# AssafSinger94/dino-tracker

Measured on NVIDIA H100. Metric: query-points/sec (854x476, T=50), higher is better.
Workload: dtype f32

## Files before the change

### dino_tracker_b200/csrc/inference.cu

```cuda
#include <algorithm>
#include <vector>

#include "common.cuh"
#include "corr.cuh"
#include "head.cuh"
#include "sample.cuh"
#include "xwin.cuh"

namespace dtk {

constexpr int TC2_BM_ROWS = 256;

__global__ void sample_query_kernel(const float* __restrict__ tpc, int T, int C, int P, int h, int w, PointAffine pa,
                                    const float* __restrict__ qp, float* __restrict__ desc, float* __restrict__ dnorm) {
  int n = blockIdx.x;
  float x = __fadd_rn(__fmul_rn(pa.aw, qp[n * 3 + 0]), pa.bw);
  float y = __fadd_rn(__fmul_rn(pa.ah, qp[n * 3 + 1]), pa.bh);
  int tq = (int)qp[n * 3 + 2];
  tq = min(max(tq, 0), T - 1);
  TriCorners c = tri_setup(x, y, 0.f, 2, h, w);
  sample_point(tpc, C, P, c, tq, -1, desc + (size_t)n * C, dnorm + n);
}

__global__ void index_traj_kernel(const int* __restrict__ grp_frame, const int* __restrict__ grp_row0,
                                  const int* __restrict__ grp_map0, int n_groups, int n_maps, int T,
                                  int* __restrict__ out_index, float* __restrict__ traj) {
  int j = blockIdx.x * blockDim.x + threadIdx.x;
  if (j >= n_maps) return;
  const int lo = last_le(n_groups, j, grp_map0);
  int n = grp_row0[lo] + (j - grp_map0[lo]);
  int t = grp_frame[lo];
  out_index[j] = n * T + t;
  traj[((size_t)n * T + t) * 3 + 2] = (float)t;
}

__global__ void traj_cos_kernel(const float* __restrict__ tpc, int T, int C, int P, int h, int w, PointAffine pa,
                                const float* __restrict__ traj, const float* __restrict__ qp,
                                float* __restrict__ cos_out) {
  extern __shared__ __align__(16) float sm[];
  __shared__ float nrm[2];
  __shared__ float red[SAMPLE_THREADS / 32];
  const int n = blockIdx.y, i = blockIdx.x;
  int tq = (int)qp[n * 3 + 2];
  tq = min(max(tq, 0), T - 1);
  for (int which = 0; which < 2; ++which) {
    const float* pt = traj + ((size_t)n * T + (which == 0 ? tq : i)) * 3;
    float x = __fadd_rn(__fmul_rn(pa.aw, pt[0]), pa.bw);
    float y = __fadd_rn(__fmul_rn(pa.ah, pt[1]), pa.bh);
    TriCorners c = tri_setup(x, y, pt[2], T, h, w);
    sample_point(tpc, C, P, c, c.z0, c.z1, sm + which * C, nrm + which);
    __syncthreads();
  }
  const float nq = fmaxf(nrm[0], 1e-8f), ni = fmaxf(nrm[1], 1e-8f);
  float acc = 0.f;
  for (int c = threadIdx.x; c < C; c += SAMPLE_THREADS) acc = fmaf(__fdiv_rn(sm[c], nq), __fdiv_rn(sm[C + c], ni), acc);
  acc = warp_sum(acc);
  if ((threadIdx.x & 31) == 0) red[threadIdx.x >> 5] = acc;
  __syncthreads();
  if (threadIdx.x == 0) {
    float s = 0.f;
    for (int k = 0; k < SAMPLE_THREADS / 32; ++k) s += red[k];
    cos_out[(size_t)n * T + i] = s;
  }
}

constexpr int ANCHOR_LIST_THREADS = 256;
__global__ void __launch_bounds__(ANCHOR_LIST_THREADS)
anchor_lists_kernel(const float* __restrict__ cos_sims, int N, int T, float th, int* __restrict__ cnt,
                    int* __restrict__ qlist) {
  const int a = blockIdx.x;
  int base = 0;
  for (int n0 = 0; n0 < N; n0 += ANCHOR_LIST_THREADS) {
    const int n = n0 + threadIdx.x;
    const bool v = n < N && cos_sims[(size_t)n * T + a] >= th;
    int total;
    const int rank = block_rank<ANCHOR_LIST_THREADS>(v, &total);
    if (v) qlist[(size_t)a * N + base + rank] = n;
    base += total;
    __syncthreads();
  }
  if (threadIdx.x == 0) cnt[a] = base;
}

struct AnchorItem { int a, slot, i, n; };
__device__ __forceinline__ AnchorItem anchor_item(int j, int lo, int T, const int* __restrict__ qlist, int N,
                                                  const int* __restrict__ grp_frame, const int* __restrict__ grp_map0,
                                                  const int* __restrict__ grp_item0) {
  AnchorItem it;
  it.a = grp_frame[lo];
  const int uu = grp_item0[lo] + (j - grp_map0[lo]);
  it.slot = uu / T; it.i = uu - it.slot * T;
  it.n = qlist[(size_t)it.a * N + it.slot];
  return it;
}

struct NoAnchor {};
__device__ __forceinline__ int slot_frame(int z, int i0, int a) { return z == 0 ? a : i0 + z - 1; }
__device__ __forceinline__ int slot_frame(int z, int i0, NoAnchor) { return i0 + z - 1; }
struct SetSample { TriCorners c; int f0, f1; };
template <class Anchor>
__device__ __forceinline__ SetSample frame_set_sample(const float* __restrict__ pt, int i, int T, int frame_batch, int h, int w,
                                                      const PointAffine& pa, Anchor a) {
  const int i0 = (i / frame_batch) * frame_batch, e = min(i0 + frame_batch, T);
  float x = __fadd_rn(__fmul_rn(pa.aw, pt[0]), pa.bw);
  float y = __fadd_rn(__fmul_rn(pa.ah, pt[1]), pa.bh);
  SetSample s;
  s.c = tri_setup(x, y, (float)(i - i0 + 1), e - i0 + 1, h, w);
  s.f0 = slot_frame(s.c.z0, i0, a);
  s.f1 = s.c.z1 < 0 ? -1 : slot_frame(s.c.z1, i0, a);
  return s;
}

__global__ void sample_anchor_kernel(const float* __restrict__ tpc, int T, int C, int P, int h, int w, PointAffine pa,
                                     const float* __restrict__ traj, const int* __restrict__ qlist, int N,
                                     const int* __restrict__ grp_frame, const int* __restrict__ grp_map0,
                                     const int* __restrict__ grp_item0, int n_groups, int frame_batch,
                                     float* __restrict__ desc, float* __restrict__ dnorm, int* __restrict__ out_index,
                                     __half* __restrict__ desc_hi, __half* __restrict__ desc_lo) {
  const int j = blockIdx.x;
  const AnchorItem it = anchor_item(j, last_le(n_groups, j, grp_map0), T, qlist, N, grp_frame, grp_map0, grp_item0);
  const SetSample s = frame_set_sample(traj + ((size_t)it.n * T + it.i) * 3, it.i, T, frame_batch, h, w, pa, it.a);
  sample_point(tpc, C, P, s.c, s.f0, s.f1, desc + (size_t)j * C, dnorm + j, desc_hi ? desc_hi + (size_t)j * C : nullptr,
               desc_lo ? desc_lo + (size_t)j * C : nullptr);
  if (threadIdx.x == 0) out_index[j] = (it.n * T + it.a) * T + it.i;
}

__device__ __forceinline__ float quant_desc(const __half* hi, const __half* lo, int C, const float* norm, int8_t* q, float* fac) {
  __syncthreads();
  if (threadIdx.x >= 32) return 0.f;
  const float nrm = *norm;
  return xw_quant_row([&](int k) {
    const uint2 a = *reinterpret_cast<const uint2*>(hi + k), b = *reinterpret_cast<const uint2*>(lo + k);
    const float2 a0 = __half22float2(*reinterpret_cast<const __half2*>(&a.x)), a1 = __half22float2(*reinterpret_cast<const __half2*>(&a.y));
    const float2 b0 = __half22float2(*reinterpret_cast<const __half2*>(&b.x)), b1 = __half22float2(*reinterpret_cast<const __half2*>(&b.y));
    return make_float4(a0.x + b0.x, a0.y + b0.y, a1.x + b1.x, a1.y + b1.y);
  }, C, nrm, q, fac);
}

__global__ void sample_unique_kernel(const float* __restrict__ tpc, int T, int C, int P, int h, int w, PointAffine pa,
                                     const float* __restrict__ traj, int frame_batch, __half* __restrict__ u_hi,
                                     __half* __restrict__ u_lo, float* __restrict__ u_norm, int* __restrict__ u_flag,
                                     int8_t* __restrict__ u_q8, float* __restrict__ u_fac, float* __restrict__ u_rho) {
  const int u = blockIdx.x;
  const SetSample s = frame_set_sample(traj + (size_t)u * 3, u % T, T, frame_batch, h, w, pa, NoAnchor{});
  bool slot0 = false;
#pragma unroll
  for (int k = 0; k < 4; ++k) slot0 = slot0 || (s.c.z0 == 0 && s.c.tok[k] >= 0 && s.c.wxy[k][0] != 0.f);
  if (threadIdx.x == 0) u_flag[u] = slot0 ? 1 : 0;
  if (slot0) return;
  sample_point(tpc, C, P, s.c, s.f0, s.f1, nullptr, u_norm + u, u_hi + (size_t)u * C, u_lo + (size_t)u * C);
  if (u_q8) {
    const float r = quant_desc(u_hi + (size_t)u * C, u_lo + (size_t)u * C, C, u_norm + u, u_q8 + (size_t)u * C, u_fac + u);
    if (threadIdx.x == 0) u_rho[u] = r;
  }
}

__global__ void anchor_scalars_kernel(int T, const int* __restrict__ qlist, int N, const int* __restrict__ grp_frame,
                                      const int* __restrict__ grp_row0, const int* __restrict__ grp_map0,
                                      const int* __restrict__ grp_item0, int n_groups, int n_maps, int n_unique, int chunk_row0,
                                      const float* __restrict__ u_norm, const int* __restrict__ u_flag,
                                      const float* __restrict__ u_rho, const float* __restrict__ rho_f, float eps_slack, bool with_eps,
                                      int* __restrict__ out_index, int* __restrict__ arow, float* __restrict__ dnorm,
                                      float* __restrict__ desc_eps) {
  const int j = blockIdx.x * blockDim.x + threadIdx.x;
  if (j >= n_maps) return;
  const int lo = last_le(n_groups, j, grp_map0);
  const AnchorItem it = anchor_item(j, lo, T, qlist, N, grp_frame, grp_map0, grp_item0);
  const size_t u = (size_t)it.n * T + it.i;
  out_index[j] = (it.n * T + it.a) * T + it.i;
  const int r0 = grp_row0[lo];
  arow[j] = r0 < n_unique ? r0 + (j - grp_map0[lo]) : chunk_row0 + j;
  if (u_flag[u]) return;
  dnorm[j] = u_norm[u];
  if (with_eps) desc_eps[j] = xw_eps_s8(u_rho[u], rho_f[it.a], eps_slack);
}

__global__ void gather_anchor_kernel(const float* __restrict__ tpc, int T, int C, int P, int h, int w, PointAffine pa,
                                     const float* __restrict__ traj, const int* __restrict__ qlist, int N,
                                     const int* __restrict__ grp_frame, const int* __restrict__ grp_row0,
                                     const int* __restrict__ grp_map0, const int* __restrict__ grp_item0, int n_groups,
                                     int n_unique, int map_lo, int frame_batch, const __half* __restrict__ u_hi,
                                     const __half* __restrict__ u_lo, const int* __restrict__ u_flag,
                                     float* __restrict__ dnorm, __half* __restrict__ desc_hi,
                                     __half* __restrict__ desc_lo, const int8_t* __restrict__ u_q8,
                                     const float* __restrict__ u_fac, const float* __restrict__ rho_f, float eps_slack,
                                     int8_t* __restrict__ desc_q8, float* __restrict__ desc_fac,
                                     float* __restrict__ desc_eps) {
  const int j = map_lo + blockIdx.x;
  const int lo = last_le(n_groups, j, grp_map0);
  if (grp_row0[lo] < n_unique) return;
  const AnchorItem it = anchor_item(j, lo, T, qlist, N, grp_frame, grp_map0, grp_item0);
  const size_t u = (size_t)it.n * T + it.i;
  if (!u_flag[u]) {
    const uint4* sh = reinterpret_cast<const uint4*>(u_hi + u * C);
    const uint4* sl = reinterpret_cast<const uint4*>(u_lo + u * C);
    uint4* dh = reinterpret_cast<uint4*>(desc_hi + (size_t)j * C);
    uint4* dl = reinterpret_cast<uint4*>(desc_lo + (size_t)j * C);
    for (int k = threadIdx.x; k < C / 8; k += blockDim.x) { dh[k] = __ldg(sh + k); dl[k] = __ldg(sl + k); }
    if (desc_q8) {
      const uint4* sq = reinterpret_cast<const uint4*>(u_q8 + u * C);
      uint4* dq = reinterpret_cast<uint4*>(desc_q8 + (size_t)j * C);
      for (int k = threadIdx.x; k < C / 16; k += blockDim.x) dq[k] = __ldg(sq + k);
      if (threadIdx.x == 0) desc_fac[j] = u_fac[u];
    }
    return;
  }
  const SetSample s = frame_set_sample(traj + u * 3, it.i, T, frame_batch, h, w, pa, it.a);
  sample_point(tpc, C, P, s.c, s.f0, s.f1, nullptr, dnorm + j, desc_hi + (size_t)j * C, desc_lo + (size_t)j * C);
  if (desc_q8) {
    const float r = quant_desc(desc_hi + (size_t)j * C, desc_lo + (size_t)j * C, C, dnorm + j, desc_q8 + (size_t)j * C, desc_fac + j);
    if (threadIdx.x == 0) desc_eps[j] = xw_eps_s8(r, rho_f[it.a], eps_slack);
  }
}

constexpr int OCC_THREADS = 256;
__global__ void occlusion_kernel(const float* __restrict__ traj, const float* __restrict__ cos_sims,
                                 const float* __restrict__ anchors, int T, float anchor_th, float cos_th,
                                 uint8_t* __restrict__ occ) {
  extern __shared__ float sm[];
  float* med = sm;
  int* alist = reinterpret_cast<int*>(sm + T);
  float* ax = sm + 2 * T;
  float* ay = sm + 3 * T;
  const int lane = threadIdx.x & 31, warp = threadIdx.x >> 5, nw = OCC_THREADS / 32;
  float* col = sm + 4 * T + warp * T;
  __shared__ int M;
  __shared__ float th_s;
  const int n = blockIdx.x;
  if (threadIdx.x == 0) {
    int m = 0;
    for (int a = 0; a < T; ++a)
      if (cos_sims[(size_t)n * T + a] >= anchor_th) {
        alist[m] = a;
        ax[m] = traj[((size_t)n * T + a) * 3 + 0];
        ay[m] = traj[((size_t)n * T + a) * 3 + 1];
        ++m;
      }
    M = m;
  }
  __syncthreads();
  const int m = M, want = (m - 1) / 2;
  for (int i = warp; i < T; i += nw) {
    for (int p = lane; p < m; p += 32) {
      const float* g = anchors + (((size_t)n * T + alist[p]) * T + i) * 2;
      float dx = __fsub_rn(g[0], ax[p]), dy = __fsub_rn(g[1], ay[p]);
      col[p] = sqrtf(__fadd_rn(__fmul_rn(dx, dx), __fmul_rn(dy, dy)));
    }
    __syncwarp();
    for (int p = lane; p < m; p += 32) {
      const float dp = col[p];
      int rank = 0;
      for (int q = 0; q < m; ++q) {
        float dq = col[q];
        rank += (dq < dp) || (dq == dp && q < p);
      }
      if (rank == want) med[i] = dp;
    }
    __syncwarp();
  }
  __syncthreads();
  if (threadIdx.x == 0) {
    float th = -INFINITY;
    for (int p = 0; p < m; ++p) th = fmaxf(th, med[alist[p]]);
    th_s = th;
  }
  __syncthreads();
  for (int i = threadIdx.x; i < T; i += blockDim.x)
    occ[(size_t)n * T + i] = (m > 0 && (med[i] > th_s || cos_sims[(size_t)n * T + i] < cos_th)) ? 1 : 0;
}

struct GroupBuf {
  std::vector<int> v;
  int cap, n;
  bool overflow = false;
  explicit GroupBuf(int c) : v((size_t)5 * c), cap(c), n(0) {}
  void clear() { n = 0; }
  void push(int frame, int row0, int m, int map0, int item0) {
    if (n >= cap) { overflow = true; return; }
    v[n] = frame; v[cap + n] = row0; v[2 * cap + n] = m; v[3 * cap + n] = map0; v[4 * cap + n] = item0; ++n;
  }
};

struct ChunkMeta { int used, maxm, n_groups; bool no_thin; int n_gathered, gather_lo, gather_hi; };
constexpr int XW_INPLACE_PAD_DIV = 16;
constexpr int XW_INPLACE_MIN_ROWS = TC2_BM_ROWS - TC2_BM_ROWS / (XW_INPLACE_PAD_DIV + 1);
struct AnchorRows { const int* qlist; const unsigned char* qflag; int gather_row0, ring, ring_stride; };
static bool plan_chunks(int kind, int T, int N, const int* cnt, int ch_all, int gcap, std::vector<ChunkMeta>& metas,
                        std::vector<int>& plan_host, int align = 1, int first_cap = 0, const AnchorRows* rows = nullptr) {
  int ch = ch_all;
  metas.clear(); plan_host.clear();
  GroupBuf gb(gcap);
  int n_gathered = 0, gather_lo = 0, gather_hi = 0;
  auto commit_chunk = [&](int used) {
    bool no_thin = true;
    int maxm = 0;
    for (int k = 0; k < gb.n; ++k) {
      no_thin = no_thin && gb.v[2 * gb.cap + k] > STREAM_MAX_M;
      maxm = std::max(maxm, gb.v[2 * gb.cap + k]);
    }
    metas.push_back(ChunkMeta{used, maxm, gb.n, no_thin, n_gathered, gather_lo, gather_hi});
    plan_host.insert(plan_host.end(), gb.v.begin(), gb.v.end());
    n_gathered = gather_lo = gather_hi = 0;
  };
  auto push_span = [&](int a, int map0, int m, int item0) {
    if (!rows) { gb.push(a, map0, m, map0, item0); return; }
    const int* ql = rows->qlist + (size_t)a * N;
    const int chunk_row0 = rows->gather_row0 + (int)(metas.size() % rows->ring) * rows->ring_stride;
    const int s0 = item0 / T, s1 = (item0 + m) / T;
    int gs = -1;
    auto close_gathered = [&](int s_end) {
      if (gs < 0) return;
      const int gm = (s_end - gs) * T, gmap = map0 + (gs - s0) * T;
      gb.push(a, chunk_row0 + gmap, gm, gmap, gs * T);
      if (n_gathered == 0) gather_lo = gmap;
      n_gathered += gm; gather_hi = gmap + gm;
      gs = -1;
    };
    for (int s = s0; s < s1;) {
      const bool flagged = rows->qflag[ql[s]] != 0;
      int e = s + 1;
      while (!flagged && e < s1 && ql[e] == ql[e - 1] + 1 && !rows->qflag[ql[e]]) ++e;
      const int r = (e - s) * T, pad = (r + TC2_BM_ROWS - 1) / TC2_BM_ROWS * TC2_BM_ROWS - r;
      if (!flagged && (long long)pad * XW_INPLACE_PAD_DIV <= r) {
        close_gathered(s);
        gb.push(a, ql[s] * T, r, map0 + (s - s0) * T, s * T);
      } else if (gs < 0) {
        gs = s;
      }
      s = e;
    }
    close_gathered(s1);
  };
  if (kind == 0) {
    int t = 0, row = 0;
    while (t < T) {
      gb.clear();
      int used = 0;
      while (t < T && used < ch && gb.n < gcap) {
        int m = N - row;
        if (m > ch - used) m = ch - used;
        gb.push(t, row, m, used, 0);
        used += m; row += m;
        if (row == N) { row = 0; ++t; }
      }
      commit_chunk(used);
    }
  } else {
    int a = 0;
    long long item = 0;
    while (a < T) {
      gb.clear();
      int used = 0;
      ch = (metas.empty() && first_cap > 0 && first_cap < ch_all) ? first_cap : ch_all;
      while (a < T && used < ch && gb.n < gcap) {
        long long tot = (long long)cnt[a] * T;
        long long m = tot - item;
        if (m > ch - used) {
          m = (long long)((ch - used) / align) * align;
          if (m == 0 && used > 0) break;
          if (m == 0) m = align;
        }
        if (m > 0) {
          push_span(a, used, (int)m, (int)item);
          used += (int)m; item += m;
        }
        if (item >= tot) { item = 0; ++a; }
      }
      if (used == 0) break;
      commit_chunk(used);
    }
  }
  return !gb.overflow;
}

struct CellPlan {
  std::vector<int> v;
  std::vector<size_t> first;
  std::vector<int> tiles;
  int max_m = 0;
};
static void plan_cells(int T, int gcap, const std::vector<ChunkMeta>& metas, const std::vector<int>& plan_host, CellPlan& cp) {
  const int nb = (T + XW_MAX_CELL - 1) / XW_MAX_CELL, rb = (T + nb - 1) / nb;
  cp.v.clear(); cp.first.assign(1, 0); cp.tiles.clear(); cp.max_m = 0;
  std::vector<int> r0, mm, fr, gr, ar;
  for (size_t k = 0; k < metas.size(); ++k) {
    const int* gb = plan_host.data() + k * 5 * gcap;
    r0.clear(); mm.clear(); fr.clear(); gr.clear(); ar.clear();
    int pre = 0;
    for (int g = 0; g < metas[k].n_groups; ++g) {
      const int frame = gb[g], row0 = gb[gcap + g], m = gb[2 * gcap + g], map0 = gb[3 * gcap + g];
      cp.tiles.push_back(pre);
      pre += (m + TC2_BM_ROWS - 1) / TC2_BM_ROWS;
      for (int s0 = 0; s0 < m; s0 += T)
        for (int b = 0; b < T; b += rb) {
          const int cm = std::min(rb, T - b);
          r0.push_back(map0 + s0 + b); mm.push_back(cm); fr.push_back(frame); gr.push_back(g); ar.push_back(row0 + s0 + b);
          cp.max_m = std::max(cp.max_m, cm);
        }
    }
    for (int g = metas[k].n_groups; g <= gcap; ++g) cp.tiles.push_back(pre);
    const size_t n = r0.size();
    cp.v.insert(cp.v.end(), r0.begin(), r0.end());
    cp.v.insert(cp.v.end(), mm.begin(), mm.end());
    cp.v.insert(cp.v.end(), fr.begin(), fr.end());
    cp.v.insert(cp.v.end(), gr.begin(), gr.end());
    cp.v.insert(cp.v.end(), ar.begin(), ar.end());
    cp.first.push_back(cp.first.back() + n);
  }
}

struct InferAsync {
  cudaStream_t side;
  cudaEvent_t fork, join, sample[2], gemm[2];
};
static int g_overlap_mode = -1;
struct InferAsyncSlot { InferAsync ia; int state; };
static InferAsync* infer_async() {
  static PerDev<InferAsyncSlot> slots;
  if (g_overlap_mode == 0) return nullptr;
  InferAsyncSlot& slot = slots.get();
  InferAsync& ia = slot.ia;
  if (slot.state == 0) {
    slot.state = -1;
    if (cudaStreamCreateWithFlags(&ia.side, cudaStreamNonBlocking) != cudaSuccess) return nullptr;
    cudaEvent_t* evs[] = {&ia.fork, &ia.join, &ia.sample[0], &ia.sample[1], &ia.gemm[0], &ia.gemm[1]};
    for (cudaEvent_t* ev : evs)
      if (cudaEventCreateWithFlags(ev, cudaEventDisableTiming) != cudaSuccess) return nullptr;
    slot.state = 1;
  }
  return slot.state == 1 ? &ia : nullptr;
}

constexpr int XW_RING = 4;
constexpr int XW_PROBE_MAPS = 4096;
constexpr int INFER_A_COUNTED = 16;
constexpr int XW_CNT_CHUNK = 4, XW_CNT_A = XW_CNT_CHUNK * XW_RING, XW_CNT_MINNORM = XW_CNT_A + INFER_A_COUNTED;
struct XwAsync {
  int state;
  cudaEvent_t sample[XW_RING], done[XW_RING], freed[XW_RING];
  int* host_cnt;
};
static XwAsync* xw_async() {
  static PerDev<XwAsync> slots;
  XwAsync& xa = slots.get();
  if (xa.state == 0) {
    xa.state = -1;
    for (int k = 0; k < XW_RING; ++k) {
      if (cudaEventCreateWithFlags(&xa.sample[k], cudaEventDisableTiming) != cudaSuccess) return nullptr;
      if (cudaEventCreateWithFlags(&xa.done[k], cudaEventDisableTiming) != cudaSuccess) return nullptr;
      if (cudaEventCreateWithFlags(&xa.freed[k], cudaEventDisableTiming) != cudaSuccess) return nullptr;
    }
    if (cudaHostAlloc(&xa.host_cnt, (XW_CNT_MINNORM + 4) * sizeof(int), cudaHostAllocDefault) != cudaSuccess) return nullptr;
    xa.state = 1;
  }
  return xa.state == 1 ? &xa : nullptr;
}
static int g_xw_path = -1;
static int g_xw_coarse = -1;
namespace infer_stat {
enum { anchor_maps, exact_window, full_map, pipeline, full_map_by_certificate, contraction, coarse, coarse_rho_f,
       desc_in_place, desc_gathered, exact_box_cells, exact_box_tokens, count };
}
static long long g_infer_stats[infer_stat::count] = {};
constexpr int XW_S8_PROBE_QUEUE_DIV = 16;

struct AnchorChoice {
  XwAsync* xa = nullptr;
  bool xw = false;
  bool probe = false;
  bool s8 = false;

  AnchorChoice(const FeatView& fv, const dinotrk_geom& g) {
    if (fv.tensor() && disc_fits_box(g) && g_xw_path != 0) xa = xw_async();
    xw = xa != nullptr;
    probe = g_xw_path < 0;
  }
  static bool q8_rows(const FeatView& fv) { return fv.s8() && g_xw_coarse != 0 && fv.C % 16 == 0 && fv.C <= XW_S8_MAX_C; }
  void after_sync(int C, int n_counted_A, long long maps_A) {
    if (!xw) return;
    float mn;
    memcpy(&mn, xa->host_cnt + XW_CNT_MINNORM, sizeof(float));
    if (!(mn >= split_min_norm(C))) xw = false;
    if (xw && probe && n_counted_A > 0) {
      long long unc = 0;
      for (int k = 0; k < n_counted_A; ++k) unc += xa->host_cnt[XW_CNT_A + k];
      if (unc * 4 > maps_A) xw = false;
    }
  }
  int coarse_pass(const FeatView& fv, float rho_max) {
    DTK_CHECK_ARG(g_xw_coarse != 1 || !xw || fv.s8(), "infer: int8 coarse pass forced without the int8 features");
    s8 = xw && fv.s8() && g_xw_coarse != 0;
    DTK_CHECK_ARG(!s8 || (fv.C % 16 == 0 && fv.C <= XW_S8_MAX_C), "infer: int8 coarse pass needs C %% 16 == 0 and C <= %d",
                  XW_S8_MAX_C);
    if (g_xw_coarse < 0 && !(rho_max <= XW_S8_RHO_MAX)) s8 = false;
    return DINOTRK_OK;
  }
  bool probe_says_full_maps(long long by_certificate, long long queued, int maps) {
    if (by_certificate * 4 > maps) return true;
    if (s8 && g_xw_coarse < 0 && queued * XW_S8_PROBE_QUEUE_DIV > maps) s8 = false;
    return false;
  }
};

struct CorrTrackWs {
  float* maps; CorrMapsWs corr; int* hscratch;
  CorrTrackWs(Arena& ar, int total_maps, int n_groups, int C, int map_stride)
      : maps(ar.take<float>((size_t)total_maps * map_stride)), corr(ar, total_maps, n_groups, C),
        hscratch(ar.take<int>(total_maps + 1)) {}
};

struct ChunkBufs {
  float* maps; float* desc; float* norm; int* plan; float* split; int* hscratch; unsigned long long* tkeys;
  ChunkBufs() = default;
  ChunkBufs(Arena& ar, int C, int N, int P, int ms, int ch, int gcap) {
    maps = ar.take<float>((size_t)ch * ms);
    desc = ar.take<float>((size_t)ch * C);
    norm = ar.take<float>(ch);
    plan = ar.take<int>(gcap + 1);
    split = ar.take<float>(corr_tc_workspace_bytes(ch > N ? ch : N, C) / 4);
    hscratch = ar.take<int>(ch + 1);
    tkeys = ar.take<unsigned long long>((size_t)ch * cdiv(P, CORR_TILE));
  }
};

struct XwSet {
  int row0; float* norm; int* out_index; int* arow; float* eps; XwChunk xc;
  XwSet() = default;
  XwSet(Arena& ar, int row0_, float* u_norm, int P, int ch, int gcap) : row0(row0_), norm(u_norm + row0_) {
    out_index = ar.take<int>(ch);
    arow = ar.take<int>(ch);
    eps = ar.take<float>(ch);
    xc = XwChunk(ar, ch, (size_t)ch + 2, cdiv(P, XW_TILE), gcap);
  }
};

struct InferWs {
  float* descA; float* normA;
  ChunkBufs cb[2];
  int* out_index_ring[4];
  int* d_groups; int* d_cnt; int* d_qlist;
  size_t xw_rows;
  __half* u_hi; __half* u_lo; int8_t* u_q8; float* u_norm; float* u_fac; int* u_flag; float* u_rho;
  float* d_rnorms; unsigned* d_minnorm;
  XwSet xr[XW_RING];
  int cell_nb;
  int* d_cells; int* d_tiles;
  int sg_cap;
  int* d_cgrp; int* d_splan; int* d_cntA;
  InferWs(Arena& ar, int T, int C, int N, int P, int ms, int ch, int gcap, size_t max_chunks) {
    descA = ar.take<float>((size_t)N * C);
    normA = ar.take<float>(N);
    for (ChunkBufs& b : cb) b = ChunkBufs(ar, C, N, P, ms, ch, gcap);
    for (int*& r : out_index_ring) r = ar.take<int>(ch);
    d_groups = ar.take<int>(max_chunks * 5 * gcap);
    d_cnt = ar.take<int>(T);
    d_qlist = ar.take<int>((size_t)T * N);
    const int n_unique = N * T;
    xw_rows = (size_t)n_unique + (size_t)XW_RING * ch;
    u_hi = ar.take<__half>(xw_rows * C);
    u_lo = ar.take<__half>(xw_rows * C);
    u_q8 = ar.take<int8_t>(xw_rows * C);
    u_norm = ar.take<float>(xw_rows);
    u_fac = ar.take<float>(xw_rows);
    u_flag = ar.take<int>((size_t)N * T);
    u_rho = ar.take<float>((size_t)N * T);
    d_rnorms = ar.take<float>((size_t)T * P);
    d_minnorm = ar.take<unsigned>(4);
    for (int k = 0; k < XW_RING; ++k) xr[k] = XwSet(ar, n_unique + k * ch, u_norm, P, ch, gcap);
    cell_nb = (T + XW_MAX_CELL - 1) / XW_MAX_CELL;
    d_cells = ar.take<int>((size_t)N * T * cell_nb * 5 + 16);
    d_tiles = ar.take<int>(max_chunks * (gcap + 1));
    sg_cap = (int)std::min<size_t>(max_chunks * (size_t)gcap, 16384);
    d_cgrp = ar.take<int>((size_t)4 * sg_cap);
    d_splan = ar.take<int>((size_t)sg_cap + 1);
    d_cntA = ar.take<int>(64);
  }
};

struct InferCtx {
  const FeatView& fv; const dinotrk_geom& g; const dinotrk_head_weights& hw;
  InferWs& ws; cudaStream_t st;
  int T, C, N, P, ms, ch, gcap, fb;
  size_t max_chunks;
  PointAffine pa;
  std::vector<ChunkMeta> metas;
  std::vector<int> plan_host;
  int upload_plan() {
    DTK_CHECK_ARG(metas.size() <= max_chunks, "infer: chunk plan exceeds its bound (%zu > %zu)", metas.size(), max_chunks);
    if (!plan_host.empty())
      DTK_CUDA(cudaMemcpyAsync(ws.d_groups, plan_host.data(), plan_host.size() * sizeof(int), cudaMemcpyHostToDevice, st));
    return DINOTRK_OK;
  }
  struct Grp { const int *f, *r, *m, *map0, *item; };
  Grp grp_of(size_t k) const {
    const int* b = ws.d_groups + k * 5 * gcap;
    return Grp{b, b + gcap, b + 2 * gcap, b + 3 * gcap, b + 4 * gcap};
  }
};

static int infer_trajectories(InferCtx& c, const float* query_points, float* traj, int& n_counted) {
  NvtxRange nv("dinotrk.infer.A.trajectories");
  InferWs& ws = c.ws;
  const bool tensor = c.fv.tensor();
  {
    ProfRange pr(PROF_SAMPLE, c.st);
    sample_query_kernel<<<c.N, SAMPLE_THREADS, 0, c.st>>>(c.fv.tpc, c.T, c.C, c.P, c.g.h, c.g.w, c.pa, query_points, ws.descA,
                                                           ws.normA);
    DTK_LAUNCHED();
  }
  if (tensor) {
    for (int k = 0; k < 2; ++k) {
      const DescSplit a(ws.cb[k].split, c.N, c.C);
      int rc = corr_hilo(c.fv) ? launch_split_hilo(ws.descA, a.hi, c.N, c.C, c.st)
                               : launch_split_f16(ws.descA, a.hi, a.lo, (size_t)c.N * c.C, c.st);
      if (rc) return rc;
    }
  }
  plan_chunks(0, c.T, c.N, nullptr, c.ch, c.gcap, c.metas, c.plan_host);
  int rc = c.upload_plan();
  if (rc) return rc;
  for (size_t k = 0; k < c.metas.size(); ++k) {
    const ChunkMeta& cm = c.metas[k];
    const ChunkBufs& b = ws.cb[k & 1];
    const InferCtx::Grp gp = c.grp_of(k);
    {
      ProfRange pr(PROF_MISC, c.st);
      index_traj_kernel<<<cdiv(cm.used, 256), 256, 0, c.st>>>(gp.f, gp.r, gp.map0, cm.n_groups, cm.used, c.T,
                                                              ws.out_index_ring[k & 3], traj);
      DTK_LAUNCHED();
    }
    CorrAssist as;
    as.tkeys = tensor ? b.tkeys : nullptr; as.zero_word = b.hscratch; as.split_ready = tensor; as.no_thin = cm.no_thin;
    rc = launch_corr_maps(c.fv, ws.descA, c.N, ws.normA, gp.f, gp.r, gp.m, gp.map0, cm.n_groups, cm.used, cm.maxm, b.maps, c.ms,
                          b.plan, b.split, c.st, as);
    if (rc) return rc;
    rc = launch_head(b.maps, cm.used, c.ms, c.g, c.hw, ws.out_index_ring[k & 3], traj, 3, 0, nullptr, b.hscratch, c.st, as.tkeys,
                     true);
    if (rc) return rc;
    if (k < INFER_A_COUNTED)
      DTK_CUDA(cudaMemcpyAsync(ws.d_cntA + k, b.hscratch, sizeof(int), cudaMemcpyDeviceToDevice, c.st));
  }
  n_counted = (int)std::min<size_t>(c.metas.size(), INFER_A_COUNTED);
  return DINOTRK_OK;
}

struct ExactWindow {
  InferCtx& c;
  const AnchorChoice& choice;
  const CellPlan& cp;
  bool ovl;
  cudaStream_t sb;
  const float* traj;
  float* anchors;
  int q_rows = 0, q_groups = 0;

  XwCells cells_of(size_t k) const {
    XwCells x;
    const int n = (int)(cp.first[k + 1] - cp.first[k]);
    const int* base = c.ws.d_cells + 5 * cp.first[k];
    x.row0 = base; x.m = base + n; x.frame = base + 2 * n; x.group = base + 3 * n; x.arow = base + 4 * n;
    x.n_cells = n; x.max_m = cp.max_m;
    return x;
  }
  int sample(size_t k) {
    InferWs& ws = c.ws;
    const ChunkMeta& cm = c.metas[k];
    const XwSet& x = ws.xr[k % XW_RING];
    const InferCtx::Grp gp = c.grp_of(k);
    if (ovl && k >= XW_RING) DTK_CUDA(cudaStreamWaitEvent(sb, choice.xa->freed[k % XW_RING], 0));
    {
      ProfRange pr(PROF_SAMPLE, sb);
      anchor_scalars_kernel<<<cdiv(cm.used, 256), 256, 0, sb>>>(c.T, ws.d_qlist, c.N, gp.f, gp.r, gp.map0, gp.item, cm.n_groups,
                                                               cm.used, c.N * c.T, x.row0, ws.u_norm, ws.u_flag, ws.u_rho,
                                                               c.fv.q_rho, xw_s8_slack(c.C), choice.s8, x.out_index, x.arow,
                                                               x.norm, x.eps);
      DTK_LAUNCHED();
      if (cm.n_gathered > 0) {
        const size_t r0 = (size_t)x.row0;
        gather_anchor_kernel<<<cm.gather_hi - cm.gather_lo, SAMPLE_THREADS, 0, sb>>>(
            c.fv.tpc, c.T, c.C, c.P, c.g.h, c.g.w, c.pa, traj, ws.d_qlist, c.N, gp.f, gp.r, gp.map0, gp.item, cm.n_groups,
            c.N * c.T, cm.gather_lo, c.fb, ws.u_hi, ws.u_lo, ws.u_flag, x.norm, ws.u_hi + r0 * c.C, ws.u_lo + r0 * c.C, ws.u_q8,
            ws.u_fac, c.fv.q_rho, xw_s8_slack(c.C), choice.s8 ? ws.u_q8 + r0 * c.C : nullptr, ws.u_fac + r0, x.eps);
        DTK_LAUNCHED();
      }
    }
    if (ovl) DTK_CUDA(cudaEventRecord(choice.xa->sample[k % XW_RING], sb));
    return DINOTRK_OK;
  }
  int flush() {
    if (q_rows == 0) return DINOTRK_OK;
    const ChunkBufs& b = c.ws.cb[0];
    CorrAssist as;
    as.tkeys = b.tkeys; as.zero_word = b.hscratch; as.split_ready = true; as.no_thin = true; as.all_wide = true; as.small_tiles = true;
    const int* cg = c.ws.d_cgrp;
    const int sg = c.ws.sg_cap;
    int rc = launch_corr_maps(c.fv, nullptr, c.ch, b.norm, cg, cg + sg, cg + 2 * sg, cg + 3 * sg, q_groups, q_rows, q_rows,
                              b.maps, c.ms, c.ws.d_splan, b.split, c.st, as);
    if (rc) return rc;
    rc = launch_head(b.maps, q_rows, c.ms, c.g, c.hw, c.ws.out_index_ring[0], anchors, 2, 0, nullptr, b.hscratch, c.st, b.tkeys,
                     true);
    q_rows = q_groups = 0;
    return rc;
  }
  int finish(size_t j) {
    InferWs& ws = c.ws;
    XwAsync* xa = choice.xa;
    DTK_CUDA(cudaEventSynchronize(xa->done[j % XW_RING]));
    const int* cnt = xa->host_cnt + XW_CNT_CHUNK * (j % XW_RING);
    const int n_slow = cnt[0];
    g_infer_stats[infer_stat::full_map_by_certificate] += cnt[1];
    g_infer_stats[infer_stat::exact_box_tokens] += cnt[2]; g_infer_stats[infer_stat::exact_box_cells] += cnt[3];
    const ChunkMeta& cm = c.metas[j];
    const XwSet& x = ws.xr[j % XW_RING];
    const InferCtx::Grp gp = c.grp_of(j);
    DTK_CHECK_ARG(n_slow >= 0 && n_slow <= cm.used, "infer: corrupt full-map queue (%d of %d)", n_slow, cm.used);
    g_infer_stats[infer_stat::exact_window] += cm.used - n_slow; g_infer_stats[infer_stat::full_map] += n_slow;
    if (n_slow > 0) {
      if (q_rows + n_slow > c.ch || q_groups + cm.n_groups > ws.sg_cap) {
        int rc = flush();
        if (rc) return rc;
      }
      const ChunkBufs& b = ws.cb[0];
      const DescSplit d(b.split, c.ch, c.C);
      int rc = launch_xw_compact(nullptr, ws.u_hi, ws.u_lo, x.arow, x.norm, x.out_index, c.C, gp.f, gp.map0, cm.n_groups, n_slow,
                                 x.xc, nullptr, d.hi, d.lo, b.norm, ws.out_index_ring[0], ws.d_cgrp, ws.sg_cap, c.st, q_rows,
                                 q_groups, corr_hilo(c.fv));
      if (rc) return rc;
      q_rows += n_slow; q_groups += cm.n_groups;
    }
    DTK_CUDA(cudaEventRecord(xa->freed[j % XW_RING], c.st));
    return DINOTRK_OK;
  }
};

static int anchors_exact_window(InferCtx& c, AnchorChoice& choice, const float* traj, float* anchors, size_t& done) {
  InferWs& ws = c.ws;
  const cudaStream_t st = c.st;
  XwAsync* xa = choice.xa;
  CellPlan cp;
  plan_cells(c.T, c.gcap, c.metas, c.plan_host, cp);
  DTK_CHECK_ARG(cp.first.back() * 5 <= (size_t)c.N * c.T * ws.cell_nb * 5 + 16, "infer: cell plan exceeds its bound");
  if (!cp.v.empty()) DTK_CUDA(cudaMemcpyAsync(ws.d_cells, cp.v.data(), cp.v.size() * sizeof(int), cudaMemcpyHostToDevice, st));
  if (!cp.tiles.empty()) DTK_CUDA(cudaMemcpyAsync(ws.d_tiles, cp.tiles.data(), cp.tiles.size() * sizeof(int), cudaMemcpyHostToDevice, st));
  InferAsync* ia = infer_async();
  const bool ovl = ia != nullptr && c.metas.size() > 1;
  ExactWindow pipe{c, choice, cp, ovl, ovl ? ia->side : st, traj, anchors};
  if (ovl) {
    DTK_CUDA(cudaEventRecord(ia->fork, st));
    DTK_CUDA(cudaStreamWaitEvent(pipe.sb, ia->fork, 0));
  }
  int rc;
  if (!c.metas.empty() && (rc = pipe.sample(0))) return rc;
  size_t n_finished = 0;
  done = c.metas.size();
  for (size_t k = 0; k < c.metas.size(); ++k) {
    const ChunkMeta& cm = c.metas[k];
    const XwSet& x = ws.xr[k % XW_RING];
    const InferCtx::Grp gp = c.grp_of(k);
    const XwCells cells = pipe.cells_of(k);
    if (ovl) DTK_CUDA(cudaStreamWaitEvent(st, xa->sample[k % XW_RING], 0));
    const float* eps = choice.s8 ? x.eps : nullptr;
    g_infer_stats[infer_stat::desc_in_place] += cm.used - cm.n_gathered; g_infer_stats[infer_stat::desc_gathered] += cm.n_gathered;
    if ((rc = launch_xw_coarse(c.fv, ws.u_hi, (int)ws.xw_rows, ws.u_norm, gp.f, gp.r, gp.m, gp.map0, ws.d_tiles + k * (c.gcap + 1),
                               cm.n_groups, cm.used / TC2_BM_ROWS + cm.n_groups, x.xc, st, ws.d_rnorms,
                               choice.s8 ? ws.u_q8 : nullptr, ws.u_fac))) return rc;
    if ((rc = launch_xw_plan(cells, x.norm, cm.n_groups, c.g, x.xc, st, cm.used, split_min_norm(c.C), eps))) return rc;
    if ((rc = launch_xw_gemm(c.fv, c.g, ws.u_hi, ws.u_lo, (int)ws.xw_rows, cells, x.xc, st))) return rc;
    if ((rc = launch_xw_head(c.fv, c.g, c.hw, cells, x.norm, gp.map0, cm.used, x.out_index, anchors, 2, 0, x.xc, st, cm.n_groups,
                             eps)))
      return rc;
    DTK_CUDA(cudaMemcpyAsync(xa->host_cnt + XW_CNT_CHUNK * (k % XW_RING), x.xc.slow_cnt + cm.n_groups, XW_CNT_CHUNK * sizeof(int),
                             cudaMemcpyDeviceToHost, st));
    DTK_CUDA(cudaEventRecord(xa->done[k % XW_RING], st));
    if (k == 0 && choice.probe && c.metas.size() > 1) {
      if ((rc = pipe.finish(0))) return rc;
      n_finished = 1;
      if (choice.probe_says_full_maps(g_infer_stats[infer_stat::full_map_by_certificate], g_infer_stats[infer_stat::full_map], cm.used)) {
        done = 1;
        break;
      }
      g_infer_stats[infer_stat::coarse] = choice.s8 ? 1 : 0;
    }
    if (k + 1 < c.metas.size() && (rc = pipe.sample(k + 1))) return rc;
    while (n_finished + 2 <= k)
      if ((rc = pipe.finish(n_finished++))) return rc;
  }
  while (n_finished < done)
    if ((rc = pipe.finish(n_finished++))) return rc;
  if ((rc = pipe.flush())) return rc;
  if (ovl) {
    DTK_CUDA(cudaEventRecord(ia->join, pipe.sb));
    DTK_CUDA(cudaStreamWaitEvent(st, ia->join, 0));
  }
  return DINOTRK_OK;
}

static int anchors_full_map(InferCtx& c, size_t k0, const float* traj, float* anchors) {
  InferWs& ws = c.ws;
  const cudaStream_t st = c.st;
  const bool tensor = c.fv.tensor();
  FeatView fv_split = c.fv;
  fv_split.hilo = nullptr;
  InferAsync* ia = infer_async();
  const bool ovl = ia != nullptr && c.metas.size() > k0 + 1;
  const cudaStream_t sb = ovl ? ia->side : st;
  if (ovl) {
    DTK_CUDA(cudaEventRecord(ia->fork, st));
    DTK_CUDA(cudaStreamWaitEvent(sb, ia->fork, 0));
  }
  auto sample = [&](size_t k) -> int {
    const ChunkMeta& cm = c.metas[k];
    const ChunkBufs& b = ws.cb[k & 1];
    const InferCtx::Grp gp = c.grp_of(k);
    if (ovl && k >= k0 + 2) DTK_CUDA(cudaStreamWaitEvent(sb, ia->gemm[k & 1], 0));
    {
      ProfRange pr(PROF_SAMPLE, sb);
      const DescSplit d(b.split, cm.used, c.C);
      __half* d_hi = tensor ? reinterpret_cast<__half*>(d.hi) : nullptr;
      __half* d_lo = tensor ? reinterpret_cast<__half*>(d.lo) : nullptr;
      sample_anchor_kernel<<<cm.used, SAMPLE_THREADS, 0, sb>>>(c.fv.tpc, c.T, c.C, c.P, c.g.h, c.g.w, c.pa, traj, ws.d_qlist, c.N,
                                                              gp.f, gp.map0, gp.item, cm.n_groups, c.fb, b.desc, b.norm,
                                                              ws.out_index_ring[k & 3], d_hi, d_lo);
      DTK_LAUNCHED();
    }
    if (ovl) DTK_CUDA(cudaEventRecord(ia->sample[k & 1], sb));
    return DINOTRK_OK;
  };
  auto head_full = [&](size_t j) {
    const ChunkBufs& b = ws.cb[j & 1];
    return launch_head(b.maps, c.metas[j].used, c.ms, c.g, c.hw, ws.out_index_ring[j & 3], anchors, 2, 0, nullptr, b.hscratch,
                       st, tensor ? b.tkeys : nullptr, true, 2);
  };
  int rc;
  if (k0 < c.metas.size() && (rc = sample(k0))) return rc;
  for (size_t k = k0; k < c.metas.size(); ++k) {
    const ChunkMeta& cm = c.metas[k];
    const ChunkBufs& b = ws.cb[k & 1];
    const InferCtx::Grp gp = c.grp_of(k);
    if (ovl) DTK_CUDA(cudaStreamWaitEvent(st, ia->sample[k & 1], 0));
    if (k >= k0 + 2 && (rc = head_full(k - 2))) return rc;
    CorrAssist as;
    as.tkeys = tensor ? b.tkeys : nullptr; as.zero_word = b.hscratch; as.split_ready = tensor; as.no_thin = cm.no_thin;
    rc = launch_corr_maps(fv_split, b.desc, cm.used, b.norm, gp.f, gp.r, gp.m, gp.map0, cm.n_groups, cm.used, cm.maxm, b.maps,
                          c.ms, b.plan, b.split, st, as);
    if (rc) return rc;
    if (ovl) DTK_CUDA(cudaEventRecord(ia->gemm[k & 1], st));
    if (k + 1 < c.metas.size() && (rc = sample(k + 1))) return rc;
    rc = launch_head(b.maps, cm.used, c.ms, c.g, c.hw, ws.out_index_ring[k & 3], anchors, 2, 0, nullptr, b.hscratch, st, as.tkeys,
                     true, 1);
    if (rc) return rc;
  }
  for (size_t j = std::max(k0, c.metas.size() >= 2 ? c.metas.size() - 2 : 0); j < c.metas.size(); ++j)
    if ((rc = head_full(j))) return rc;
  return DINOTRK_OK;
}

static int infer_anchors(InferCtx& c, const float* traj, const float* cos_sims, float anchor_th, float* anchors, int n_counted_A) {
  NvtxRange nv("dinotrk.infer.C.anchors");
  InferWs& ws = c.ws;
  const cudaStream_t st = c.st;
  const int T = c.T, N = c.N;
  {
    ProfRange pr(PROF_ANCHOR_LIST, st);
    anchor_lists_kernel<<<T, ANCHOR_LIST_THREADS, 0, st>>>(cos_sims, N, T, anchor_th, ws.d_cnt, ws.d_qlist);
    DTK_LAUNCHED();
  }
  AnchorChoice choice(c.fv, c.g);
  XwAsync* xa = choice.xa;
  if (xa) {
    int rc = launch_xw_rnorms(c.fv, ws.d_rnorms, ws.d_minnorm, st);
    if (rc) return rc;
    DTK_CUDA(cudaMemcpyAsync(xa->host_cnt + XW_CNT_MINNORM, ws.d_minnorm, sizeof(unsigned), cudaMemcpyDeviceToHost, st));
    if (n_counted_A > 0)
      DTK_CUDA(cudaMemcpyAsync(xa->host_cnt + XW_CNT_A, ws.d_cntA, (size_t)n_counted_A * sizeof(int), cudaMemcpyDeviceToHost, st));
  }
  std::vector<int> cnt(T);
  DTK_CUDA(cudaMemcpyAsync(cnt.data(), ws.d_cnt, (size_t)T * sizeof(int), cudaMemcpyDeviceToHost, st));
  std::vector<float> rho_f(c.fv.s8() ? T : 0);
  if (c.fv.s8()) DTK_CUDA(cudaMemcpyAsync(rho_f.data(), c.fv.q_rho, (size_t)T * sizeof(float), cudaMemcpyDeviceToHost, st));
  std::vector<int> qlist_h, uflag_h;
  if (choice.xw) {
    {
      ProfRange pr(PROF_SAMPLE, st);
      sample_unique_kernel<<<N * T, SAMPLE_THREADS, 0, st>>>(c.fv.tpc, T, c.C, c.P, c.g.h, c.g.w, c.pa, traj, c.fb, ws.u_hi, ws.u_lo,
                                                             ws.u_norm, ws.u_flag, AnchorChoice::q8_rows(c.fv) ? ws.u_q8 : nullptr,
                                                             ws.u_fac, ws.u_rho);
      DTK_LAUNCHED();
    }
    qlist_h.resize((size_t)T * N); uflag_h.resize((size_t)N * T);
    DTK_CUDA(cudaMemcpyAsync(qlist_h.data(), ws.d_qlist, qlist_h.size() * sizeof(int), cudaMemcpyDeviceToHost, st));
    DTK_CUDA(cudaMemcpyAsync(uflag_h.data(), ws.u_flag, uflag_h.size() * sizeof(int), cudaMemcpyDeviceToHost, st));
  }
  DTK_CUDA(cudaStreamSynchronize(st));
  choice.after_sync(c.C, n_counted_A, (long long)N * T);
  long long maps_C = 0;
  for (int a = 0; a < T; ++a) maps_C += (long long)cnt[a] * T;
  long long* stats = g_infer_stats;
  stats[infer_stat::anchor_maps] = maps_C; stats[infer_stat::exact_window] = 0; stats[infer_stat::full_map] = 0;
  stats[infer_stat::pipeline] = choice.xw ? 1 : 0; stats[infer_stat::full_map_by_certificate] = 0;
  stats[infer_stat::contraction] = c.fv.tensor() ? 1 : 0; stats[infer_stat::desc_in_place] = 0; stats[infer_stat::desc_gathered] = 0;
  stats[infer_stat::exact_box_cells] = 0; stats[infer_stat::exact_box_tokens] = 0;
  float rho_max = 0.f;
  for (float r : rho_f) rho_max = std::max(rho_max, r);
  int rc = choice.coarse_pass(c.fv, rho_max);
  if (rc) return rc;
  unsigned bits;
  memcpy(&bits, &rho_max, sizeof(bits));
  stats[infer_stat::coarse] = choice.s8 ? 1 : 0; stats[infer_stat::coarse_rho_f] = bits;
  const int probe_cap = choice.probe ? std::max(T, (XW_PROBE_MAPS / T) * T) : 0;
  size_t k0 = 0;
  if (choice.xw) {
    std::vector<unsigned char> qflag(N, 0);
    for (size_t u = 0; u < uflag_h.size(); ++u)
      if (uflag_h[u]) qflag[u / T] = 1;
    const AnchorRows rows{qlist_h.data(), qflag.data(), N * T, XW_RING, c.ch};
    DTK_CHECK_ARG(plan_chunks(1, T, N, cnt.data(), c.ch, c.gcap, c.metas, c.plan_host, T, probe_cap, &rows),
                  "infer: a chunk of the anchor phase has more than %d groups", c.gcap);
    if ((rc = c.upload_plan())) return rc;
    if ((rc = anchors_exact_window(c, choice, traj, anchors, k0))) return rc;
    if (k0 == c.metas.size()) return DINOTRK_OK;
    stats[infer_stat::pipeline] = 0; stats[infer_stat::coarse] = 0;
    plan_chunks(1, T, N, cnt.data(), c.ch, c.gcap, c.metas, c.plan_host, T, probe_cap);
  } else {
    plan_chunks(1, T, N, cnt.data(), c.ch, c.gcap, c.metas, c.plan_host);
  }
  if ((rc = c.upload_plan())) return rc;
  return anchors_full_map(c, k0, traj, anchors);
}

}

using namespace dtk;

extern "C" {

int dinotrk_infer_set_path(int path) {
  DTK_CHECK_ARG(path >= -1 && path <= 1, "infer_set_path: -1 (automatic), 0 (full-map GEMM + head) or 1 (coarse pass + exact window)");
  g_xw_path = path;
  return DINOTRK_OK;
}

int dinotrk_infer_set_coarse(int mode) {
  DTK_CHECK_ARG(mode >= -1 && mode <= 1, "infer_set_coarse: -1 (automatic), 0 (fp16) or 1 (int8)");
  g_xw_coarse = mode;
  return DINOTRK_OK;
}

int dinotrk_infer_last_stats(long long* out, int n) {
  DTK_CHECK_ARG(out && n >= 4, "infer_last_stats: need at least 4 slots");
  for (int i = 0; i < (n < infer_stat::count ? n : infer_stat::count); ++i) out[i] = g_infer_stats[i];
  return DINOTRK_OK;
}

static int infer_chunk_maps(int chunk_maps) { return chunk_maps > 0 ? chunk_maps : 4096; }
static int infer_chunk_eff(int chunk_maps, int T) { const int c = infer_chunk_maps(chunk_maps); return c > T ? c : T; }
static int infer_gcap(int T, int ch) { return T + 2 + 2 * (ch / XW_INPLACE_MIN_ROWS + 1); }
static size_t infer_max_chunks(int T, int N, size_t ch) {
  size_t cap = (ch / (size_t)T) * (size_t)T;
  if (cap < (size_t)T) cap = T;
  return ((size_t)N * T * T + cap - 1) / cap + 2;
}

size_t dinotrk_infer_max_chunks(int T, int N, int chunk_maps) {
  const size_t ch = (size_t)infer_chunk_maps(chunk_maps);
  return ((size_t)N * T * T + ch - 1) / ch + 2;
}

int dinotrk_infer_plan(int kind, int T, int N, const int* anchor_counts, int chunk_maps, int* groups, int* meta,
                       int max_chunks, int* n_chunks) {
  DTK_CHECK_ARG((kind == 0 || kind == 1) && T > 0 && N >= 0 && n_chunks, "infer_plan: bad arguments");
  DTK_CHECK_ARG(kind == 0 || anchor_counts, "infer_plan: kind 1 needs the per-frame anchor counts");
  const int ch = infer_chunk_maps(chunk_maps), gcap = T + 2;
  std::vector<ChunkMeta> metas;
  std::vector<int> plan_host;
  plan_chunks(kind, T, N, anchor_counts, ch, gcap, metas, plan_host);
  *n_chunks = (int)metas.size();
  DTK_CHECK_ARG((int)metas.size() <= max_chunks || (!groups && !meta), "infer_plan: %zu chunks, room for %d", metas.size(), max_chunks);
  if (groups) std::copy(plan_host.begin(), plan_host.end(), groups);
  if (meta)
    for (size_t k = 0; k < metas.size(); ++k) {
      meta[4 * k] = metas[k].used; meta[4 * k + 1] = metas[k].maxm; meta[4 * k + 2] = metas[k].n_groups;
      meta[4 * k + 3] = metas[k].no_thin ? 1 : 0;
    }
  return DINOTRK_OK;
}

int dinotrk_infer_anchor_gcap(int T, int chunk_maps) { return T > 0 ? infer_gcap(T, infer_chunk_eff(chunk_maps, T)) : 0; }

int dinotrk_infer_plan_anchors(int T, int N, const int* anchor_counts, const int* qlist, const unsigned char* query_flag,
                               int chunk_maps, int probe, int* groups, int* meta, int max_chunks, int* n_chunks) {
  DTK_CHECK_ARG(T > 0 && N >= 0 && anchor_counts && qlist && query_flag && n_chunks, "infer_plan_anchors: bad arguments");
  for (int a = 0; a < T; ++a) {
    DTK_CHECK_ARG(anchor_counts[a] >= 0 && anchor_counts[a] <= N, "infer_plan_anchors: count of frame %d out of range", a);
    for (int k = 0; k < anchor_counts[a]; ++k)
      DTK_CHECK_ARG(qlist[(size_t)a * N + k] >= 0 && qlist[(size_t)a * N + k] < N, "infer_plan_anchors: query out of range");
  }
  const int ch = infer_chunk_eff(chunk_maps, T), gcap = infer_gcap(T, ch);
  const AnchorRows rows{qlist, query_flag, N * T, XW_RING, ch};
  std::vector<ChunkMeta> metas;
  std::vector<int> plan_host;
  const bool fits = plan_chunks(1, T, N, anchor_counts, ch, gcap, metas, plan_host, T,
                                probe ? std::max(T, (XW_PROBE_MAPS / T) * T) : 0, &rows);
  DTK_CHECK_ARG(fits, "infer_plan_anchors: a chunk has more than %d groups", gcap);
  *n_chunks = (int)metas.size();
  DTK_CHECK_ARG((int)metas.size() <= max_chunks || (!groups && !meta), "infer_plan_anchors: %zu chunks, room for %d", metas.size(), max_chunks);
  if (groups) std::copy(plan_host.begin(), plan_host.end(), groups);
  if (meta)
    for (size_t k = 0; k < metas.size(); ++k) {
      meta[5 * k] = metas[k].used; meta[5 * k + 1] = metas[k].maxm; meta[5 * k + 2] = metas[k].n_groups;
      meta[5 * k + 3] = metas[k].no_thin ? 1 : 0; meta[5 * k + 4] = metas[k].n_gathered;
    }
  return DINOTRK_OK;
}

int dinotrk_infer_set_overlap(int mode) {
  DTK_CHECK_ARG(mode >= -1 && mode <= 1, "infer_set_overlap: mode must be -1 (default), 0 or 1");
  g_overlap_mode = mode;
  return DINOTRK_OK;
}

size_t dinotrk_corr_track_workspace_bytes(int total_maps, int n_groups, int C, const dinotrk_geom* g) {
  if (!g) return 0;
  return align_up(layout_end<CorrTrackWs>(total_maps, n_groups, C, dinotrk_map_stride(g)), 256) + 1024;
}

int dinotrk_corr_track(const dinotrk_features* feat, const dinotrk_geom* g,
                       const dinotrk_head_weights* hw, const float* desc, const float* desc_norm,
                       const int* grp_frame, const int* grp_row0, const int* grp_m, const int* grp_map0,
                       int n_groups, int total_maps, int max_group_m, const int* out_index, float* out,
                       int out_stride, int out_mode, void* workspace, size_t workspace_bytes, void* stream) {
  DTK_CHECK_ARG(feat && feat->tpc && feat->norms && g && hw && desc && desc_norm && grp_frame && grp_row0 && grp_m &&
                grp_map0 && out, "corr_track: null pointer");
  const int C = feat->C;
  DTK_CHECK_ARG(feat->T > 0 && C > 0 && C % 4 == 0 && n_groups >= 0 && total_maps >= 0, "corr_track: bad sizes");
  DTK_CHECK_ARG((feat->hi == nullptr) == (feat->lo == nullptr), "corr_track: hi and lo must be given together");
  DTK_CHECK_ARG(workspace && workspace_bytes >= dinotrk_corr_track_workspace_bytes(total_maps, n_groups, C, g),
                "corr_track: workspace too small");
  if (total_maps == 0) return DINOTRK_OK;
  const int ms = dinotrk_map_stride(g);
  Arena ar(workspace);
  const CorrTrackWs ws(ar, total_maps, n_groups, C, ms);
  cudaStream_t st = (cudaStream_t)stream;
  int rc = launch_corr_maps(make_view(*feat, *g), desc, total_maps, desc_norm, grp_frame, grp_row0, grp_m, grp_map0,
                            n_groups, total_maps, max_group_m, ws.maps, ms, ws.corr.plan, ws.corr.split, st);
  if (rc) return rc;
  return launch_head(ws.maps, total_maps, ms, *g, *hw, out_index, out, out_stride, out_mode, nullptr, ws.hscratch, st);
}


size_t dinotrk_infer_workspace_bytes(int T, int C, const dinotrk_geom* g, int N, int chunk_maps) {
  if (!g) return 0;
  const int ch = infer_chunk_eff(chunk_maps, T);
  const size_t end = layout_end<InferWs>(T, C, N, g->h * g->w, dinotrk_map_stride(g), ch, infer_gcap(T, ch),
                                         infer_max_chunks(T, N, (size_t)ch));
  return align_up(end, 256) + 25088;
}

int dinotrk_traj_cos_sims(const float* tpc, int T, int C, const dinotrk_geom* g, const float* traj,
                          const float* query_points, int N, float* cos_sims, void* workspace,
                          size_t workspace_bytes, void* stream) {
  (void)workspace; (void)workspace_bytes;
  DTK_CHECK_ARG(tpc && g && traj && query_points && cos_sims, "traj_cos_sims: null pointer");
  DTK_CHECK_ARG(T > 0 && C > 0 && C % 4 == 0 && N >= 0, "traj_cos_sims: bad sizes");
  if (N == 0) return DINOTRK_OK;
  size_t smem = (size_t)2 * C * sizeof(float);
  static PerDev<size_t> attr_dev;
  size_t& attr = attr_dev.get();
  if (smem > 48 * 1024 && smem > attr) {
    DTK_CUDA(cudaFuncSetAttribute(traj_cos_kernel, cudaFuncAttributeMaxDynamicSharedMemorySize, (int)smem));
    attr = smem;
  }
  ProfRange pr(PROF_COS, (cudaStream_t)stream);
  traj_cos_kernel<<<dim3(T, N), SAMPLE_THREADS, smem, (cudaStream_t)stream>>>(
      tpc, T, C, g->h * g->w, g->h, g->w, make_point_affine(*g), traj, query_points, cos_sims);
  DTK_LAUNCHED();
  return DINOTRK_OK;
}

int dinotrk_occlusion(const float* traj, const float* cos_sims, const float* anchors, int N, int T,
                      float anchor_th, float cos_th, uint8_t* occ, void* stream) {
  DTK_CHECK_ARG(traj && cos_sims && anchors && occ && N >= 0 && T > 0, "occlusion: bad args");
  if (N == 0) return DINOTRK_OK;
  size_t smem = (size_t)(4 + OCC_THREADS / 32) * T * sizeof(float);
  DTK_CHECK_ARG(smem <= 200 * 1024, "occlusion: T=%d too large", T);
  static PerDev<size_t> attr_dev;
  size_t& attr = attr_dev.get();
  if (smem > 48 * 1024 && smem > attr) {
    DTK_CUDA(cudaFuncSetAttribute(occlusion_kernel, cudaFuncAttributeMaxDynamicSharedMemorySize, (int)smem));
    attr = smem;
  }
  ProfRange pr(PROF_OCCLUSION, (cudaStream_t)stream);
  occlusion_kernel<<<N, OCC_THREADS, smem, (cudaStream_t)stream>>>(traj, cos_sims, anchors, T, anchor_th, cos_th, occ);
  DTK_LAUNCHED();
  return DINOTRK_OK;
}

int dinotrk_infer(const dinotrk_features* feat, const dinotrk_geom* g,
                  const dinotrk_head_weights* hw, const float* query_points, int N, float anchor_th, float cos_th,
                  int frame_batch, int start_phase, int stop_after, int chunk_maps, float* traj, float* cos_sims,
                  float* anchors,
                  uint8_t* occ, void* workspace, size_t workspace_bytes, void* stream) {
  DTK_CHECK_ARG(feat && feat->tpc && feat->norms && g && hw && query_points && traj, "infer: null pointer");
  const int T = feat->T, C = feat->C;
  DTK_CHECK_ARG(T > 0 && C > 0 && C % 4 == 0 && N >= 0, "infer: bad sizes");
  DTK_CHECK_GRID(*g, "infer");
  DTK_CHECK_ARG((feat->hi == nullptr) == (feat->lo == nullptr), "infer: hi and lo must be given together");
  const FeatView fv = make_view(*feat, *g);
  DTK_CHECK_ARG(start_phase >= 0 && start_phase <= stop_after && stop_after <= 3,
                "infer: need 0 <= start_phase <= stop_after <= 3");
  DTK_CHECK_ARG((stop_after < 1 || cos_sims) && (stop_after < 2 || anchors) && (stop_after < 3 || occ),
                "infer: missing output buffer for the requested phases");
  DTK_CHECK_ARG(workspace && workspace_bytes >= dinotrk_infer_workspace_bytes(T, C, g, N, chunk_maps),
                "infer: workspace too small (%zu < %zu)", workspace_bytes,
                dinotrk_infer_workspace_bytes(T, C, g, N, chunk_maps));
  if (N == 0) return DINOTRK_OK;
  const int P = g->h * g->w, ms = dinotrk_map_stride(g);
  const int ch = infer_chunk_eff(chunk_maps, T);
  const int fb = frame_batch > 0 ? (frame_batch < T ? frame_batch : T) : T;
  const int gcap = infer_gcap(T, ch);
  const size_t max_chunks = infer_max_chunks(T, N, (size_t)ch);
  Arena ar(workspace);
  InferWs ws(ar, T, C, N, P, ms, ch, gcap, max_chunks);
  DTK_CHECK_ARG(ws.xw_rows <= 0x7fffffffu, "infer: %zu descriptor rows exceed the row index", ws.xw_rows);
  InferCtx c{fv, *g, *hw, ws, (cudaStream_t)stream, T, C, N, P, ms, ch, gcap, fb, max_chunks, make_point_affine(*g)};

  int rc, n_counted_A = 0;
  if (start_phase <= 0 && (rc = infer_trajectories(c, query_points, traj, n_counted_A))) return rc;
  if (stop_after < 1) return DINOTRK_OK;
  if (start_phase <= 1) {
    NvtxRange nv("dinotrk.infer.B.cos_sims");
    if ((rc = dinotrk_traj_cos_sims(feat->tpc, T, C, g, traj, query_points, N, cos_sims, nullptr, 0, stream))) return rc;
  }
  if (stop_after < 2) return DINOTRK_OK;
  if (start_phase <= 2 && (rc = infer_anchors(c, traj, cos_sims, anchor_th, anchors, n_counted_A))) return rc;
  if (stop_after < 3) return DINOTRK_OK;
  NvtxRange nv("dinotrk.infer.D.occlusion");
  return dinotrk_occlusion(traj, cos_sims, anchors, N, T, anchor_th, cos_th, occ, stream);
}

}
```

### dino_tracker_b200/csrc/xwin.cu

```cuda
#include <cuda_fp16.h>

#include "common.cuh"
#include "corr.cuh"
#include "head.cuh"
#include "tcgemm.cuh"
#include "xwin.cuh"

namespace dtk {

constexpr int XW_GEMM_BN = 2 * XW_TILE;

template <class Acc>
struct CoarseEpi {
  static constexpr bool kFragment = true;
  static constexpr bool kS8 = std::is_same<Acc, int>::value;
  const float* rnorms;
  const float* desc_norm;
  const int* grp_map0;
  unsigned long long* key1;
  float* max2;
  int n_tiles, P;

  struct Pre { float2 col; float dv; int map0; };
  __device__ __forceinline__ Pre begin(const TcTile& tl, int t, int r) const {
    const float* rn = rnorms + (size_t)tl.batch * P;
    const int c0 = tl.n0 + t, c1 = c0 + XW_TILE;
    const int rr = r + 8 * ((threadIdx.x & 3) >> 1);
    Pre p;
    p.col = make_float2(c0 < P ? __ldg(rn + c0) : 0.f, c1 < P ? __ldg(rn + c1) : 0.f);
    p.dv = rr < tl.m ? __ldg(desc_norm + tl.row0 + rr) : 0.f;
    p.map0 = __ldg(grp_map0 + tl.g);
    return p;
  }
  static __device__ __forceinline__ float as_float(Acc a) {
    if constexpr (kS8) return __int_as_float(a); else return a;
  }
  static __device__ __forceinline__ Acc from_float(float v) {
    if constexpr (kS8) return __float_as_int(v); else return v;
  }
  template <bool EDGE>
  __device__ __forceinline__ void fold_max(float (&m1)[2], int kh, const float* cols, int n0, int fc,
                                           Acc (&acc)[XW_GEMM_BN / 2]) const {
#pragma unroll
    for (int ii = 0; ii < XW_TILE / 8; ++ii) {
      const int i = kh * XW_TILE / 8 + ii;
      const float2 rnv = tc::lds_f2(tc::smem_u32(cols + fc + 8 * i));
      const int col = n0 + 8 * i + fc;
      const bool ok0 = !EDGE || col < P, ok1 = !EDGE || col + 1 < P;
#pragma unroll
      for (int h = 0; h < 2; ++h) {
        const float a = ok0 ? (float)acc[4 * i + 2 * h] * rnv.x : -INFINITY;
        const float b = ok1 ? (float)acc[4 * i + 2 * h + 1] * rnv.y : -INFINITY;
        acc[4 * i + 2 * h] = from_float(a);
        acc[4 * i + 2 * h + 1] = from_float(b);
        m1[h] = fmaxf(m1[h], fmaxf(a, b));
      }
    }
  }
  __device__ __forceinline__ void scan(float m1, int h, int kh, const Acc (&acc)[XW_GEMM_BN / 2], float& pos,
                                       float& m2) const {
    pos = 0.f;
    m2 = -INFINITY;
#pragma unroll
    for (int ii = XW_TILE / 8 - 1; ii >= 0; --ii) {
      const int i = kh * XW_TILE / 8 + ii;
#pragma unroll
      for (int j = 1; j >= 0; --j)
        asm("{\n\t.reg .pred p;\n\t"
            "setp.eq.f32 p, %2, %3;\n\t"
            "@p fma.rn.f32 %0, %0, 0f3B000000, %4;\n\t"
            "@!p max.f32 %1, %1, %2;\n\t}"
            : "+f"(pos), "+f"(m2)
            : "f"(as_float(acc[4 * i + 2 * h + j])), "f"(m1), "f"((float)(8 * i + j + 1)));
    }
  }
  __device__ __forceinline__ void fragment(const TcTile& tl, int r, int fc, Acc (&acc)[XW_GEMM_BN / 2], const float* cols,
                                           const Pre& pre) const {
    const int q = threadIdx.x & 3, n0 = tl.n0;
    const bool edge = n0 + XW_GEMM_BN > P;
    float o1, o2;
    int otok;
#pragma unroll
    for (int kh = 0; kh < 2; ++kh) {
      float m1[2] = {-INFINITY, -INFINITY};
      if (edge) fold_max<true>(m1, kh, cols, n0, fc, acc);
      else fold_max<false>(m1, kh, cols, n0, fc, acc);
#pragma unroll
      for (int h = 0; h < 2; ++h) {
#pragma unroll
        for (int sh = 1; sh <= 2; sh <<= 1) m1[h] = fmaxf(m1[h], __shfl_xor_sync(0xffffffffu, m1[h], sh));
        float pos, m2;
        scan(m1[h], h, kh, acc, pos, m2);
        const int ip = (int)pos;
        int tok = ip ? n0 + fc + ip - 1 : 0x7fffffff;
        int cnt = (ip != 0) + ((float)ip != pos);
#pragma unroll
        for (int sh = 1; sh <= 2; sh <<= 1) {
          tok = min(tok, __shfl_xor_sync(0xffffffffu, tok, sh));
          cnt += __shfl_xor_sync(0xffffffffu, cnt, sh);
          m2 = fmaxf(m2, __shfl_xor_sync(0xffffffffu, m2, sh));
        }
        if ((q & 1) == kh && (q >> 1) == h) {
          o1 = m1[h];
          o2 = cnt > 1 ? m1[h] : m2;
          otok = tok;
        }
      }
    }
    const int rr = r + 8 * (q >> 1), nt = n0 / XW_TILE + (q & 1);
    if (rr >= tl.m || nt >= n_tiles) return;
    const float rdn = kS8 ? pre.dv : __fdividef(1.f, fmaxf(pre.dv, XW_MIN_NORM));
    const size_t off = (size_t)(pre.map0 + rr) * n_tiles + nt;
    key1[off] = ((unsigned long long)__float_as_uint(fmaxf(o1 * rdn, 0.f)) << 32) | (unsigned)(0x7fffffff - otok);
    max2[off] = fmaxf(o2 * rdn, 0.f);
  }
};

__global__ void xw_rnorm_kernel(const float* __restrict__ norms, float* __restrict__ rnorms, size_t n, unsigned* __restrict__ min_bits) {
  float mn = INFINITY;
  for (size_t i = (size_t)blockIdx.x * blockDim.x + threadIdx.x; i < n; i += (size_t)gridDim.x * blockDim.x) {
    const float v = norms[i];
    rnorms[i] = __fdiv_rn(1.f, fmaxf(v, XW_MIN_NORM));
    mn = fminf(mn, v);
  }
#pragma unroll
  for (int o = 16; o > 0; o >>= 1) mn = fminf(mn, __shfl_xor_sync(0xffffffffu, mn, o));
  if ((threadIdx.x & 31) == 0) atomicMin(min_bits, __float_as_uint(fmaxf(mn, 0.f)));
}

int launch_xw_rnorms(const FeatView& fv, float* rnorms, unsigned* min_bits, cudaStream_t st) {
  const size_t n = (size_t)fv.T * fv.P;
  DTK_CUDA(cudaMemsetAsync(min_bits, 0x7f, sizeof(unsigned), st));
  ProfRange pr(PROF_XW_PLAN, st);
  xw_rnorm_kernel<<<num_sms() * 4, 256, 0, st>>>(fv.norms, rnorms, n, min_bits);
  DTK_LAUNCHED();
  return DINOTRK_OK;
}

int launch_xw_coarse(const FeatView& fv, const void* desc_hi, int desc_rows, const float* desc_norm, const int* grp_frame,
                     const int* grp_row0, const int* grp_m, const int* grp_map0, const int* tile_start, int n_groups,
                     int max_tiles, const XwChunk& xc, cudaStream_t st, const float* rnorms, const void* desc_q8,
                     const float* desc_fac) {
  static_assert(XW_GEMM_BN == 256 && XW_TILE == 128, "one m64n256 GEMM N tile = two 128-token key tiles (CoarseEpi::fragment)");
  TcProblem pb{grp_frame, grp_row0, grp_m, tile_start, n_groups, fv.P, fv.C};
  if (desc_q8) {
    DTK_CHECK_ARG(fv.s8() && fv.C % 16 == 0 && fv.C <= XW_S8_MAX_C, "int8 coarse pass: needs the int8 features, C %% 16 == 0 "
                  "and C <= %d", XW_S8_MAX_C);
    CoarseEpi<int> epi{fv.q_fac, desc_fac, grp_map0, xc.key1, xc.max2, cdiv(fv.P, XW_TILE), fv.P};
    return tc_launch<TcMode::S8, CoarseEpi<int>, XW_GEMM_BN, true>({desc_q8, nullptr, (uint64_t)desc_rows, 0, fv.q8, nullptr,
                                                                    (uint64_t)fv.T, 0}, pb, max_tiles, epi, st, PROF_XW_COARSE);
  }
  CoarseEpi<float> epi{rnorms, desc_norm, grp_map0, xc.key1, xc.max2, cdiv(fv.P, XW_TILE), fv.P};
  return tc_launch<TcMode::F16, CoarseEpi<float>, XW_GEMM_BN, true>({desc_hi, nullptr, (uint64_t)desc_rows, 0, fv.hi, nullptr,
                                                                     (uint64_t)fv.T, 0}, pb, max_tiles, epi, st, PROF_XW_COARSE);
}

constexpr int PLAN_WARPS = 8;
template <int KPL>
__global__ void __launch_bounds__(PLAN_WARPS * 32)
xw_cand_kernel(int n_maps, const float* __restrict__ desc_norm, float min_norm, int n_groups, int n_tiles,
               const unsigned long long* __restrict__ key1, const float* __restrict__ eps_map,
               const float* __restrict__ max2, int* __restrict__ cand, int* __restrict__ pinfo, int* __restrict__ slow_cnt) {
  const int lane = threadIdx.x & 31;
  const int gw = blockIdx.x * PLAN_WARPS + (threadIdx.x >> 5), nw = gridDim.x * PLAN_WARPS;
  if (gw == 0)
    for (int i = lane; i <= n_groups + 3; i += 32) slow_cnt[i] = 0;
  for (int map = gw; map < n_maps; map += nw) {
    const unsigned long long* k1 = key1 + (size_t)map * n_tiles;
    const float* k2 = max2 + (size_t)map * n_tiles;
    unsigned long long kk[KPL] = {};
    float v2[KPL] = {};
#pragma unroll
    for (int q = 0; q < KPL; ++q) {
      const int t = lane + 32 * q;
      if (t < n_tiles) { kk[q] = __ldg(k1 + t); v2[q] = __ldg(k2 + t); }
    }
    unsigned long long gk = kk[0];
#pragma unroll
    for (int q = 1; q < KPL; ++q) gk = gk > kk[q] ? gk : kk[q];
#pragma unroll
    for (int o = 16; o > 0; o >>= 1) { unsigned long long t = __shfl_xor_sync(0xffffffffu, gk, o); gk = t > gk ? t : gk; }
    const float gmax = __uint_as_float((unsigned)(gk >> 32));
    const int ptok = 0x7fffffff - (int)(gk & 0xffffffffu);
    const float eps = eps_map ? eps_map[map] : XW_EPS;
    const float th = gmax - 2.f * eps;
    bool amb = false;
    int ncand = 0;
#pragma unroll
    for (int q = 0; q < KPL; ++q) {
      const int t = lane + 32 * q;
      const bool in = t < n_tiles;
      const bool isc = in && __uint_as_float((unsigned)(kk[q] >> 32)) >= th;
      const unsigned cm = __ballot_sync(0xffffffffu, isc);
      amb = amb || __any_sync(0xffffffffu, in && v2[q] >= th);
      const int rank = ncand + __popc(cm & ((1u << lane) - 1u));
      if (isc && rank < XW_MAX_CAND) cand[(size_t)map * XW_MAX_CAND + rank] = 0x7fffffff - (int)(kk[q] & 0xffffffffu);
      ncand += __popc(cm);
    }
    amb = amb || ncand > XW_MAX_CAND || !(gmax > 4.f * eps) || !(desc_norm[map] >= min_norm);
    if (lane >= ncand && lane < XW_MAX_CAND) cand[(size_t)map * XW_MAX_CAND + lane] = -1;
    if (lane == 0) pinfo[map] = amb ? -1 - ptok : ptok;
  }
}

__global__ void __launch_bounds__(PLAN_WARPS * 32)
xw_cell_kernel(XwCells cells, int w, const int* __restrict__ cand, const int* __restrict__ pinfo, int* __restrict__ stat,
               int* __restrict__ cell_of, int2* __restrict__ box_org, int4* __restrict__ box_ext, int* __restrict__ box_cnt) {
  __shared__ short s_r[PLAN_WARPS][XW_MAX_CELL], s_c[PLAN_WARPS][XW_MAX_CELL];
  __shared__ unsigned char s_ok[PLAN_WARPS][XW_MAX_CELL];
  const int lane = threadIdx.x & 31, wid = threadIdx.x >> 5;
  const int gw = blockIdx.x * PLAN_WARPS + wid, nw = gridDim.x * PLAN_WARPS;
  for (int cell = gw; cell < cells.n_cells; cell += nw) {
    const int row0 = cells.row0[cell], m = cells.m[cell];
    int nv = 0;
    for (int r = lane; r < m; r += 32) {
      const int pi = __ldg(pinfo + row0 + r);
      const int ptok = pi >= 0 ? pi : -1 - pi;
      s_r[wid][r] = (short)(ptok / w);
      s_c[wid][r] = (short)(ptok - (ptok / w) * w);
      s_ok[wid][r] = pi >= 0 ? 1 : 0;
      nv += pi >= 0 ? 1 : 0;
      cell_of[row0 + r] = cell;
    }
    __syncwarp();
#pragma unroll
    for (int o = 16; o > 0; o >>= 1) nv += __shfl_xor_sync(0xffffffffu, nv, o);
    int med_r = -1, med_c = -1;
    if (nv > 0) {
      const int want = (nv - 1) / 2;
      for (int r = lane; r < m; r += 32) {
        if (!s_ok[wid][r]) continue;
        int rk_r = 0, rk_c = 0;
        const int vr = s_r[wid][r], vc = s_c[wid][r];
        for (int q = 0; q < m; ++q) {
          if (!s_ok[wid][q]) continue;
          rk_r += (s_r[wid][q] < vr) || (s_r[wid][q] == vr && q < r);
          rk_c += (s_c[wid][q] < vc) || (s_c[wid][q] == vc && q < r);
        }
        if (rk_r == want) med_r = vr;
        if (rk_c == want) med_c = vc;
      }
#pragma unroll
      for (int o = 16; o > 0; o >>= 1) {
        med_r = max(med_r, __shfl_xor_sync(0xffffffffu, med_r, o));
        med_c = max(med_c, __shfl_xor_sync(0xffffffffu, med_c, o));
      }
    }
    int n_fit = 0, lo_r = INT_MAX, hi_r = INT_MIN, lo_c = INT_MAX, hi_c = INT_MIN;
    for (int r = lane; r < m; r += 32) {
      const int map = row0 + r;
      bool fit = s_ok[wid][r] != 0;
      int mr0 = INT_MAX, mr1 = INT_MIN, mc0 = INT_MAX, mc1 = INT_MIN;
      if (fit) {
        const int4 cd = __ldg(reinterpret_cast<const int4*>(cand) + map);
        const int ct[4] = {cd.x, cd.y, cd.z, cd.w};
#pragma unroll
        for (int q = 0; q < XW_MAX_CAND; ++q)
          if (ct[q] >= 0) {
            const int tr = ct[q] / w, tc_ = ct[q] - tr * w;
            fit = fit && abs(tr - med_r) <= XW_SLACK && abs(tc_ - med_c) <= XW_SLACK;
            mr0 = min(mr0, tr); mr1 = max(mr1, tr); mc0 = min(mc0, tc_); mc1 = max(mc1, tc_);
          }
      }
      stat[map] = fit ? 0 : 1;
      n_fit += fit ? 1 : 0;
      if (fit) { lo_r = min(lo_r, mr0); hi_r = max(hi_r, mr1); lo_c = min(lo_c, mc0); hi_c = max(hi_c, mc1); }
    }
#pragma unroll
    for (int o = 16; o > 0; o >>= 1) {
      n_fit += __shfl_xor_sync(0xffffffffu, n_fit, o);
      lo_r = min(lo_r, __shfl_xor_sync(0xffffffffu, lo_r, o)); hi_r = max(hi_r, __shfl_xor_sync(0xffffffffu, hi_r, o));
      lo_c = min(lo_c, __shfl_xor_sync(0xffffffffu, lo_c, o)); hi_c = max(hi_c, __shfl_xor_sync(0xffffffffu, hi_c, o));
    }
    if (lane == 0) {
      const int org_r = med_r - XW_BOX / 2, org_c = med_c - XW_BOX / 2;
      box_org[cell] = n_fit > 0 ? make_int2(org_r, org_c) : make_int2(0, INT_MIN);
      if (n_fit > 0) {
        const int4 e = make_int4(lo_r - WM / 2 - org_r, lo_c - WM / 2 - org_c, hi_r - lo_r + WM, hi_c - lo_c + WM);
        box_ext[cell] = e;
        atomicAdd(box_cnt, e.z * e.w);
        atomicAdd(box_cnt + 1, 1);
      }
    }
    __syncwarp();
  }
}

int launch_xw_plan(const XwCells& cells, const float* desc_norm, int n_groups, const dinotrk_geom& g, const XwChunk& xc,
                   cudaStream_t st, int n_maps, float min_norm, const float* eps) {
  static_assert(XW_MAX_CAND == 4, "candidates are read as one int4");
  const int n_tiles = cdiv(g.h * g.w, XW_TILE);
  DTK_CHECK_GRID(g, "exact-window path");
  static_assert(DTK_GRID_MAX_TOKENS <= 256 * XW_TILE, "xw_cand_kernel keeps at most 8 keys per lane");
  DTK_CHECK_ARG(cells.max_m <= XW_MAX_CELL, "exact-window path: cell of %d rows", cells.max_m);
  if (cells.n_cells <= 0 || n_maps <= 0) return DINOTRK_OK;
  ProfRange pr(PROF_XW_PLAN, st);
  int grid = cdiv(n_maps, PLAN_WARPS);
  if (grid > num_sms() * 8) grid = num_sms() * 8;
  auto cand_kernel = n_tiles <= 64 ? xw_cand_kernel<2> : n_tiles <= 128 ? xw_cand_kernel<4> : xw_cand_kernel<8>;
  cand_kernel<<<grid, PLAN_WARPS * 32, 0, st>>>(n_maps, desc_norm, min_norm, n_groups, n_tiles, xc.key1, eps, xc.max2, xc.cand, xc.pinfo, xc.slow_cnt);
  DTK_LAUNCHED();
  grid = cdiv(cells.n_cells, PLAN_WARPS);
  if (grid > num_sms() * 8) grid = num_sms() * 8;
  xw_cell_kernel<<<grid, PLAN_WARPS * 32, 0, st>>>(cells, g.w, xc.cand, xc.pinfo, xc.stat, xc.cell_of, xc.box_org, xc.box_ext,
                                                   xc.slow_cnt + n_groups + 2);
  DTK_LAUNCHED();
  return DINOTRK_OK;
}

constexpr int XW_EXT_MIN = WM;
constexpr int XW_NW = XW_BOX - XW_EXT_MIN + 1;
constexpr int XW_PART_TOK = 128;
constexpr int XW_PART_ROWS = XW_PART_TOK / XW_EXT_MIN;
constexpr int XW_EPI_ROWS = 16;
constexpr int XW_EPI_PITCH = 40;

template <bool HILO>
struct XwTokMaps { CUtensorMap m[HILO ? 1 : 2][XW_NW][XW_PART_ROWS]; };

template <int MB, bool HILO>
struct XwCfg {
  static constexpr int kBK = 32;
  static constexpr int kRow = 2 * kBK;
  static constexpr int kTokRow = HILO ? 2 * kRow : kRow;
  static constexpr int kBoxes = HILO ? 1 : 2;
  static constexpr int kDescBytes = MB * kRow;
  static constexpr int kSlotBytes = XW_PART_TOK * kTokRow;
  static constexpr int kParts = MB == 64 ? 2 : 1;
  static constexpr int kTokOff = 2 * kDescBytes;
  static constexpr int kStageBytes = kTokOff + kParts * kBoxes * kSlotBytes;
  static constexpr int kStages = MB == 64 ? 5 : 6;
  static constexpr int kBarBytes = 256;
  static constexpr int kEpiBytes = 8 * XW_EPI_ROWS * XW_EPI_PITCH * 4;
  static constexpr int kSmem = kStages * kStageBytes + 1024 + kBarBytes + kEpiBytes;
  static_assert(2 * kStages * 8 <= kBarBytes, "barriers");
  static_assert(kSmem <= 227 * 1024, "shared-memory ring too large");
  static_assert(kTokOff % 1024 == 0 && kSlotBytes % 1024 == 0 && kStageBytes % 1024 == 0,
                "token boxes must start 1024-byte aligned");
};

template <int MB>
struct XwExt {
  int y, x, bh, bw, n;
  XwExt() = default;
  __device__ __forceinline__ XwExt(const int4* __restrict__ box_ext, int cell) {
    const int4 e = box_ext ? __ldg(box_ext + cell) : make_int4(0, 0, XW_BOX, XW_BOX);
    y = e.x; x = e.y; bh = e.z; bw = e.w;
    const int rp = XW_PART_TOK / max(bw, 1);
    n = ok() ? (bh + rp - 1) / rp : 0;
    if (MB == 64) n += n & 1;
  }
  __device__ __forceinline__ bool ok() const {
    return y >= 0 && x >= 0 && bh >= XW_EXT_MIN && bw >= XW_EXT_MIN && y + bh <= XW_BOX && x + bw <= XW_BOX;
  }
  __device__ __forceinline__ int rows(int i) const { return bh / n + (i < bh % n ? 1 : 0); }
  __device__ __forceinline__ int row(int i) const { return y + i * (bh / n) + min(i, bh % n); }
};

template <int MB, bool HILO>
__device__ __forceinline__ void xw_part(uint8_t* smem, uint64_t* full, uint64_t* empty, float* epi, int& stage, int& phase, int KB,
                                        uint32_t d_off, uint32_t t_off, uint32_t t_half, float* __restrict__ xbox, int map0,
                                        int r0, int m, int ntok, int bw, int col0) {
  using Cfg = XwCfg<MB, HILO>;
  constexpr int N = XW_PART_TOK;
  const int warp = threadIdx.x >> 5, lane = threadIdx.x & 31, t = threadIdx.x & 127;
  float acc[N / 2];
#pragma unroll
  for (int i = 0; i < N / 2; ++i) acc[i] = 0.f;
  int prev = -1;
  for (int kb = 0; kb < KB; ++kb) {
    tc::mbar_wait(&full[stage], phase);
    tc::wgmma_fence();
    const uint32_t sd = tc::smem_u32(smem + stage * Cfg::kStageBytes) + d_off;
    const uint32_t st = tc::smem_u32(smem + stage * Cfg::kStageBytes) + t_off;
#pragma unroll
    for (int ks = 0; ks < Cfg::kBK / 16; ++ks) {
      const uint32_t koff = ks * 32;
      const uint64_t d_hi = tc::smem_desc_sw64(sd + koff), d_lo = tc::smem_desc_sw64(sd + Cfg::kDescBytes + koff);
      const uint64_t t_hi = HILO ? tc::smem_desc_sw128(st + koff) : tc::smem_desc_sw64(st + koff);
      const uint64_t t_lo = HILO ? tc::smem_desc_sw128(st + Cfg::kRow + koff) : tc::smem_desc_sw64(st + t_half + koff);
      tc::wgmma_ss<false, N>(acc, d_lo, t_hi, 1u);
      tc::wgmma_ss<false, N>(acc, d_hi, t_lo, 1u);
      tc::wgmma_ss<false, N>(acc, d_hi, t_hi, 1u);
    }
    tc::wgmma_commit();
    tc::wgmma_wait<1>();
    if (prev >= 0 && t == 0) tc::mbar_arrive(&empty[prev]);
    prev = stage;
    if (++stage == Cfg::kStages) { stage = 0; phase ^= 1; }
  }
  tc::wgmma_wait<0>();
  tc::reg_fence(acc);
  if (prev >= 0 && t == 0) tc::mbar_arrive(&empty[prev]);
  const int rw = r0 + (warp & 3) * 16, fr = lane >> 2, fc = 2 * (lane & 3);
  float* buf = epi + (warp & 7) * XW_EPI_ROWS * XW_EPI_PITCH;
  float* dst = xbox + (size_t)(map0 + rw) * XW_COLS + col0;
  const int nr = min(m - rw, XW_EPI_ROWS);
#pragma unroll
  for (int q = 0; q < N / 32; ++q) {
    if (32 * q >= ntok || nr <= 0) break;
#pragma unroll
    for (int ii = 0; ii < 4; ++ii)
#pragma unroll
      for (int h = 0; h < 2; ++h)
        *reinterpret_cast<float2*>(buf + (fr + 8 * h) * XW_EPI_PITCH + 8 * ii + fc) =
            make_float2(acc[4 * (4 * q + ii) + 2 * h], acc[4 * (4 * q + ii) + 2 * h + 1]);
    __syncwarp();
    const int j = 32 * q + lane, y = j / bw, off = y * XW_BOX + (j - y * bw);
    if (j < ntok)
      for (int k = 0; k < nr; ++k) dst[(size_t)k * XW_COLS + off] = buf[k * XW_EPI_PITCH + lane];
    __syncwarp();
  }
}

template <int MB, bool HILO>
__global__ void __launch_bounds__(TC_THREADS, 1)
xw_gemm_kernel(const __grid_constant__ CUtensorMap tmD_hi, const __grid_constant__ CUtensorMap tmD_lo,
               const __grid_constant__ XwTokMaps<HILO> tok, XwCells cells, const int2* __restrict__ box_org,
               const int4* __restrict__ box_ext, float* __restrict__ xbox, int K) {
  using Cfg = XwCfg<MB, HILO>;
  extern __shared__ uint8_t smem_raw[];
  uint8_t* smem = reinterpret_cast<uint8_t*>((reinterpret_cast<uintptr_t>(smem_raw) + 1023) & ~(uintptr_t)1023);
  uint64_t* full = reinterpret_cast<uint64_t*>(smem + Cfg::kStages * Cfg::kStageBytes);
  uint64_t* empty = full + Cfg::kStages;
  float* epi = reinterpret_cast<float*>(smem + Cfg::kStages * Cfg::kStageBytes + Cfg::kBarBytes);

  const int warp = threadIdx.x >> 5, wg = threadIdx.x >> 7;
  const int KB = (K + Cfg::kBK - 1) / Cfg::kBK;

  if (threadIdx.x == 0) {
    tc::prefetch_tmap(&tmD_hi); tc::prefetch_tmap(&tmD_lo);
    for (int s = 0; s < Cfg::kStages; ++s) { tc::mbar_init(&full[s], 1); tc::mbar_init(&empty[s], 2); }
    tc::mbar_fence_init();
  }
  __syncthreads();

  if (wg == 0) {
    tc::regs_dealloc<40>();
    if (warp == 0 && tc::elect_one()) {
      int stage = 0, phase = 0;
      for (int cell = blockIdx.x; cell < cells.n_cells; cell += gridDim.x) {
        const int2 org = box_org[cell];
        if (org.y == INT_MIN) continue;
        const XwExt<MB> e(box_ext, cell);
        const int drow = cells.arow[cell], frame = cells.frame[cell], col = org.y + e.x;
        const int wi = e.bw - XW_EXT_MIN;
        for (int p0 = 0; p0 < e.n; p0 += Cfg::kParts) {
          int tok_rows = 0;
          for (int q = 0; q < Cfg::kParts; ++q) tok_rows += e.rows(p0 + q) * e.bw;
          for (int kb = 0; kb < KB; ++kb) {
            const int k0 = kb * Cfg::kBK, kt = HILO ? 2 * k0 : k0;
            tc::mbar_wait(&empty[stage], phase ^ 1);
            uint8_t* st = smem + stage * Cfg::kStageBytes;
            tc::mbar_expect_tx(&full[stage], 2 * Cfg::kDescBytes + Cfg::kBoxes * tok_rows * Cfg::kTokRow);
            for (int q = 0; q < Cfg::kParts; ++q) {
              uint8_t* s = st + Cfg::kTokOff + q * Cfg::kBoxes * Cfg::kSlotBytes;
              const int ri = e.rows(p0 + q) - 1, row = org.x + e.row(p0 + q);
              tc::tma_load_4d(&tok.m[0][wi][ri], &full[stage], s, kt, col, row, frame);
              if constexpr (!HILO) tc::tma_load_4d(&tok.m[1][wi][ri], &full[stage], s + Cfg::kSlotBytes, kt, col, row, frame);
            }
            tc::tma_load_2d(&tmD_hi, &full[stage], st, k0, drow);
            tc::tma_load_2d(&tmD_lo, &full[stage], st + Cfg::kDescBytes, k0, drow);
            if (++stage == Cfg::kStages) { stage = 0; phase ^= 1; }
          }
        }
      }
    }
  } else {
    tc::regs_alloc<232>();
    const int cw = wg - 1;
    int stage = 0, phase = 0;
    struct Meta { bool skip; XwExt<MB> e; int m, map0; };
    auto meta = [&](int cell) {
      return Meta{box_org[cell].y == INT_MIN, XwExt<MB>(box_ext, cell), cells.m[cell], cells.row0[cell]};
    };
    Meta cur;
    if (blockIdx.x < cells.n_cells) cur = meta(blockIdx.x);
    for (int cell = blockIdx.x; cell < cells.n_cells; cell += gridDim.x) {
      Meta nxt;
      if (cell + gridDim.x < cells.n_cells) nxt = meta(cell + gridDim.x);
      const XwExt<MB>& e = cur.e;
      const int m = cur.m, map0 = cur.map0;
      if (!cur.skip)
        for (int p0 = 0; p0 < e.n; p0 += Cfg::kParts) {
          if constexpr (MB == 64) {
            const int p = p0 + cw;
            xw_part<MB, HILO>(smem, full, empty, epi, stage, phase, KB, 0, Cfg::kTokOff + cw * Cfg::kBoxes * Cfg::kSlotBytes,
                              Cfg::kSlotBytes, xbox, map0, 0, m, e.rows(p) * e.bw, e.bw, xw_col(e.row(p), e.x));
          } else {
            xw_part<MB, HILO>(smem, full, empty, epi, stage, phase, KB, cw * 64 * Cfg::kRow, Cfg::kTokOff, Cfg::kSlotBytes,
                              xbox, map0, 64 * cw, m, e.rows(p0) * e.bw, e.bw, xw_col(e.row(p0), e.x));
          }
        }
      cur = nxt;
    }
  }
}

template <bool HILO>
static int xw_tok_maps(const FeatView& fv, const dinotrk_geom& g, const XwTokMaps<HILO>*& out) {
  struct Entry { const void* base[2]; uint64_t dims[4]; bool valid; XwTokMaps<HILO> maps; };
  static PerDev<Entry> cache;
  Entry& e = cache.get();
  const void* base[2] = {HILO ? fv.hilo : fv.hi, HILO ? nullptr : fv.lo};
  const uint64_t row = HILO ? (uint64_t)hilo_row(fv.C) : (uint64_t)fv.C;
  const uint64_t dims[4] = {row, (uint64_t)g.w, (uint64_t)g.h, (uint64_t)fv.T};
  if (!e.valid || memcmp(e.base, base, sizeof(base)) != 0 || memcmp(e.dims, dims, sizeof(dims)) != 0) {
    e.valid = false;
    const uint64_t strides[3] = {row * 2, (uint64_t)g.w * row * 2, (uint64_t)fv.P * row * 2};
    constexpr int BK = XwCfg<64, HILO>::kBK;
    const uint32_t ib = HILO ? 2 * BK : BK, tsw = HILO ? 128 : 2 * BK;
    for (int o = 0; o < (HILO ? 1 : 2); ++o)
      for (int wi = 0; wi < XW_NW; ++wi)
        for (int ri = 0; ri < XW_PART_ROWS; ++ri) {
          const uint32_t box[4] = {ib, (uint32_t)(XW_EXT_MIN + wi), (uint32_t)(1 + ri), 1};
          if (int rc = make_tmap_4d(&e.maps.m[o][wi][ri], base[o], dims, strides, box, TMAP_F16, tsw)) return rc;
        }
    memcpy(e.base, base, sizeof(base));
    memcpy(e.dims, dims, sizeof(dims));
    e.valid = true;
  }
  out = &e.maps;
  return DINOTRK_OK;
}

template <int MB, bool HILO>
static int run_xw_gemm(const FeatView& fv, const dinotrk_geom& g, const CUtensorMap (&tmD)[2], const XwCells& cells,
                       const XwChunk& xc, cudaStream_t st) {
  const XwTokMaps<HILO>* tok;
  if (int rc = xw_tok_maps<HILO>(fv, g, tok)) return rc;
  static PerDev<bool> attr_dev;
  bool& attr = attr_dev.get();
  if (!attr) {
    DTK_CUDA(cudaFuncSetAttribute(xw_gemm_kernel<MB, HILO>, cudaFuncAttributeMaxDynamicSharedMemorySize, XwCfg<MB, HILO>::kSmem));
    attr = true;
  }
  const int sms = num_sms();
  const int grid = cells.n_cells < sms ? cells.n_cells : sms;
  ProfRange pr(PROF_XW_GEMM, st);
  xw_gemm_kernel<MB, HILO><<<grid, TC_THREADS, XwCfg<MB, HILO>::kSmem, st>>>(tmD[0], tmD[1], *tok, cells, xc.box_org, xc.box_ext,
                                                                              xc.xbox, fv.C);
  DTK_LAUNCHED();
  return DINOTRK_OK;
}

int launch_xw_gemm(const FeatView& fv, const dinotrk_geom& g, const void* desc_hi, const void* desc_lo, int desc_rows,
                   const XwCells& cells, const XwChunk& xc, cudaStream_t st) {
  if (cells.n_cells <= 0) return DINOTRK_OK;
  DTK_CHECK_ARG(fv.C % 8 == 0 && cells.max_m <= XW_MAX_CELL, "exact-window GEMM: bad sizes");
  const bool small = cells.max_m <= 64, hilo = fv.hilo != nullptr;
  constexpr int BK = XwCfg<64, false>::kBK, SW = 2 * BK;
  CUtensorMap tmD[2];
  int rc;
  if ((rc = make_tmap_2d(&tmD[0], desc_hi, desc_rows, fv.C, small ? 64 : 128, BK, TMAP_F16, 0, SW))) return rc;
  if ((rc = make_tmap_2d(&tmD[1], desc_lo, desc_rows, fv.C, small ? 64 : 128, BK, TMAP_F16, 0, SW))) return rc;
  if (hilo) return small ? run_xw_gemm<64, true>(fv, g, tmD, cells, xc, st) : run_xw_gemm<128, true>(fv, g, tmD, cells, xc, st);
  return small ? run_xw_gemm<64, false>(fv, g, tmD, cells, xc, st) : run_xw_gemm<128, false>(fv, g, tmD, cells, xc, st);
}

constexpr int XH_WARPS = 8;
constexpr int XH_WP = 16;
constexpr int XH_WIN = WM * XH_WP;
constexpr int XH_RP = 20;
constexpr int XH_RED = 240;
constexpr int XH_ZB = 128;
constexpr int XH_RAW = 2 * XH_WIN + 4 * XH_RED + 2 * XH_ZB;
constexpr int XH_PER_WARP = XH_RAW + 4 * XH_WIN;
constexpr int XH_SMEM = XH_WARPS * XH_PER_WARP * 4;
static_assert(XH_WIN % 32 == 16 && XH_RED % 32 == 16 && WB * XH_RP <= XH_RED && WB * WB <= XH_ZB, "head buffer layout");

constexpr int XH_KEYS = 4;

struct XhGather {
  int amax;
  float dn, mout;
  unsigned ok;
};

__device__ __forceinline__ void xh_cp4(float* dst, const float* src) {
  asm volatile("cp.async.ca.shared.global [%0], [%1], 4;\n" ::"r"((unsigned)__cvta_generic_to_shared(dst)), "l"(src) : "memory");
}
__device__ __forceinline__ void xh_cp_wait() { asm volatile("cp.async.wait_all;\n" ::: "memory"); }

__device__ __forceinline__ void xh_gather(XhGather& gt, int map, int n_maps, int l, int h, int w, int P, int n_tiles,
                                          const float* __restrict__ norms, const float* __restrict__ desc_norm,
                                          const int* __restrict__ cell_frame, const int* __restrict__ cell_of,
                                          const int2* __restrict__ box_org, const int* __restrict__ stat,
                                          const int* __restrict__ cand, const unsigned long long* __restrict__ key1,
                                          const float* __restrict__ max2, const float* __restrict__ xbox,
                                          const float* __restrict__ eps_map, float* __restrict__ racc, float* __restrict__ rfn) {
  gt.amax = -1;
  gt.ok = 0;
  if (map >= n_maps) return;
  const int st = __ldg(stat + map), cell = __ldg(cell_of + map);
  const float dn = __ldg(desc_norm + map);
  const int4 cd = __ldg(reinterpret_cast<const int4*>(cand) + map);
  const float eps = eps_map ? __ldg(eps_map + map) : XW_EPS;
  const unsigned long long* k1 = key1 + (size_t)map * n_tiles;
  const float* k2 = max2 + (size_t)map * n_tiles;
  unsigned long long kk[XH_KEYS];
  float kv2[XH_KEYS];
#pragma unroll
  for (int q = 0; q < XH_KEYS; ++q) {
    const int t = l + 16 * q;
    kk[q] = t < n_tiles ? __ldg(k1 + t) : 0ull;
    kv2[q] = t < n_tiles ? __ldg(k2 + t) : 0.f;
  }
  if (st != 0) return;
  const int2 org = __ldg(box_org + cell);
  const float* fn = norms + (size_t)__ldg(cell_frame + cell) * P;
  const float* xr = xbox + (size_t)map * XW_COLS;
  const int ct[4] = {cd.x, cd.y, cd.z, cd.w};
  float best = -1.f;
  int amax = -1;
#pragma unroll
  for (int q = 0; q < XW_MAX_CAND; ++q)
    if (ct[q] >= 0) {
      const int tr = ct[q] / w, tcn = ct[q] - tr * w;
      const float v = fmaxf(corr_cos(__ldg(xr + xw_col(tr - org.x, tcn - org.y)), dn, __ldg(fn + ct[q])), 0.f);
      if (v > best || (v == best && ct[q] < amax)) { best = v; amax = ct[q]; }
    }
  const int arow = amax / w, acol = amax - arow * w;
  float mout = 0.f;
  auto fold = [&](unsigned long long k, float m2) {
    const int tk = 0x7fffffff - (int)(k & 0xffffffffu);
    const int tr = tk / w, tcn = tk - tr * w;
    const bool in_core = abs(tr - arow) <= 3 && abs(tcn - acol) <= 3;
    mout = fmaxf(mout, (in_core ? m2 : __uint_as_float((unsigned)(k >> 32))) + eps);
  };
#pragma unroll
  for (int q = 0; q < XH_KEYS; ++q)
    if (l + 16 * q < n_tiles) fold(kk[q], kv2[q]);
  for (int t = l + 16 * XH_KEYS; t < n_tiles; t += 16) fold(__ldg(k1 + t), __ldg(k2 + t));
  const int c = acol - 7 + l;
  const bool col_in = l < WM && c >= 0 && c < w;
  unsigned ok = 0;
#pragma unroll
  for (int y = 0; y < WM; ++y) {
    const int r = arow - 7 + y;
    if (col_in && r >= 0 && r < h) {
      xh_cp4(racc + y * XH_WP + l, xr + xw_col(r - org.x, c - org.y));
      xh_cp4(rfn + y * XH_WP + l, fn + r * w + c);
      ok |= 1u << y;
    }
  }
  gt.amax = amax;
  gt.dn = dn;
  gt.mout = mout;
  gt.ok = ok;
}

__device__ __forceinline__ float xh_window(const XhGather& gt, const float* __restrict__ racc, const float* __restrict__ rfn,
                                           float* __restrict__ win, int l) {
  xh_cp_wait();
  float mout = gt.mout;
#pragma unroll
  for (int y = 0; y < WM; ++y) {
    float v = 0.f;
    if ((gt.ok >> y) & 1u) {
      v = fmaxf(corr_cos(racc[y * XH_WP + l], gt.dn, rfn[y * XH_WP + l]), 0.f);
      if (!(abs(y - 7) <= 3 && abs(l - 7) <= 3)) mout = fmaxf(mout, v);
    }
    win[y * XH_WP + l] = v;
  }
  return mout;
}

__device__ __forceinline__ float xh_tap3(const float* wk, float v0, float v1, float v2) {
  return __fmaf_rn(wk[2], v2, __fmaf_rn(wk[1], v1, __fmul_rn(wk[0], v0)));
}

template <bool INTERIOR>
__device__ __forceinline__ void xh_step(int j, const float (&A0in)[WB], const float (&Sin)[WB], float (&A0out)[WB],
                                        float (&Sout)[WB], const float* __restrict__ win, float* __restrict__ red,
                                        float* __restrict__ zb, const float (&w1)[9], float b1, const float (&w2)[9], float b2,
                                        bool row_in, unsigned cmask, int l) {
  float in[3][16];
#pragma unroll
  for (int ky = 0; ky < 3; ++ky)
#pragma unroll
    for (int q = 0; q < 4; ++q) {
      const float4 v = *reinterpret_cast<const float4*>(win + (j + ky) * XH_WP + 4 * q);
      in[ky][4 * q] = v.x; in[ky][4 * q + 1] = v.y; in[ky][4 * q + 2] = v.z; in[ky][4 * q + 3] = v.w;
    }
  float hr[WH];
#pragma unroll
  for (int x = 0; x < WH; ++x) {
    float a0 = __fmaf_rn(w1[0], in[0][x], b1), a1 = __fmul_rn(w1[3], in[1][x]), a2 = __fmul_rn(w1[6], in[2][x]);
    a0 = __fmaf_rn(w1[1], in[0][x + 1], a0); a1 = __fmaf_rn(w1[4], in[1][x + 1], a1); a2 = __fmaf_rn(w1[7], in[2][x + 1], a2);
    a0 = __fmaf_rn(w1[2], in[0][x + 2], a0); a1 = __fmaf_rn(w1[5], in[1][x + 2], a1); a2 = __fmaf_rn(w1[8], in[2][x + 2], a2);
    const float a = __fadd_rn(__fadd_rn(a0, a1), a2);
    hr[x] = INTERIOR || (row_in && ((cmask >> x) & 1u)) ? fmaxf(a, 0.f) : 0.f;
  }
  if (j < WB) {
#pragma unroll
    for (int x = 0; x < WB; ++x) A0out[x] = xh_tap3(w2, hr[x], hr[x + 1], hr[x + 2]);
  }
  if (j >= 1 && j <= WB) {
#pragma unroll
    for (int x = 0; x < WB; ++x) Sout[x] = __fadd_rn(A0in[x], xh_tap3(w2 + 3, hr[x], hr[x + 1], hr[x + 2]));
  }
  if (j >= 2) {
    float* rb = red + (j & 1) * (2 * XH_RED);
#pragma unroll
    for (int x = 0; x < WB; ++x) rb[x * XH_RP + l] = __fadd_rn(Sin[x], xh_tap3(w2 + 6, hr[x], hr[x + 1], hr[x + 2]));
    __syncwarp();
    if (l < WB) {
      float p[16];
#pragma unroll
      for (int q = 0; q < 4; ++q) {
        const float4 v = *reinterpret_cast<const float4*>(rb + l * XH_RP + 4 * q);
        p[4 * q] = v.x; p[4 * q + 1] = v.y; p[4 * q + 2] = v.z; p[4 * q + 3] = v.w;
      }
      float v[8];
#pragma unroll
      for (int i = 0; i < 8; ++i) v[i] = __fadd_rn(p[i], p[i + 8]);
      const float t = __fadd_rn(__fadd_rn(__fadd_rn(v[0], v[4]), __fadd_rn(v[2], v[6])),
                                __fadd_rn(__fadd_rn(v[1], v[5]), __fadd_rn(v[3], v[7])));
      zb[(j - 2) * WB + l] = __fadd_rn(t, b2);
    }
  }
}

template <bool INTERIOR>
__device__ __forceinline__ void xh_refine(const float* __restrict__ win, float* __restrict__ red, float* __restrict__ zb,
                                          const float (&w1)[9], float b1, const float (&w2)[9], float b2, int arow, int acol,
                                          int h, int w, int l) {
  unsigned cmask = 0;
#pragma unroll
  for (int x = 0; x < WH; ++x) cmask |= (acol - 6 + x >= 0 && acol - 6 + x < w) ? 1u << x : 0u;
  float A0a[WB], Sa[WB], A0b[WB], Sb[WB];
#pragma unroll
  for (int x = 0; x < WB; ++x) { A0a[x] = 0.f; Sa[x] = 0.f; }
#pragma unroll 1
  for (int j = 0; j < WH; j += 2) {
    xh_step<INTERIOR>(j, A0a, Sa, A0b, Sb, win, red, zb, w1, b1, w2, b2, arow - 6 + j >= 0 && arow - 6 + j < h, cmask, l);
    if (j + 1 < WH)
      xh_step<INTERIOR>(j + 1, A0b, Sb, A0a, Sa, win, red, zb, w1, b1, w2, b2, arow - 5 + j >= 0 && arow - 5 + j < h, cmask, l);
  }
}

__device__ __forceinline__ void xh_sums(const HeadParams& hp, const float* __restrict__ zb, int arow, int acol, int l,
                                        float& zmax, float (&tot)[5]) {
  float z[8];
  bool valid[8];
  zmax = -INFINITY;
#pragma unroll
  for (int k = 0; k < 8; ++k) {
    const int p = l + 16 * k;
    const int y = p / WB, x = p - y * WB, r = arow - 5 + y, c = acol - 5 + x;
    valid[k] = p < WB * WB && r >= 0 && r < hp.h && c >= 0 && c < hp.w;
    z[k] = valid[k] ? zb[p] : -INFINITY;
    zmax = fmaxf(zmax, z[k]);
  }
#pragma unroll
  for (int o = 8; o > 0; o >>= 1) zmax = fmaxf(zmax, __shfl_xor_sync(0xffffffffu, zmax, o));
  float s[2][5] = {};
#pragma unroll
  for (int k = 0; k < 8; ++k) {
    const int p = l + 16 * k;
    const int y = p / WB, x = p - y * WB, r = arow - 5 + y, c = acol - 5 + x;
    const float e = valid[k] ? expf(z[k] - zmax) : 0.f;
    float (&t)[5] = s[k & 1];
    t[0] += e;
    if (valid[k] && in_disc(hp, r, c, arow, acol)) {
      t[1] += e; t[2] = fmaf(token_px(hp, c), e, t[2]); t[3] = fmaf(token_px(hp, r), e, t[3]);
    }
    t[4] += valid[k] ? 1.f : 0.f;
  }
#pragma unroll
  for (int i = 0; i < 5; ++i) {
    float v = s[0][i] + s[1][i];
#pragma unroll
    for (int o = 8; o > 0; o >>= 1) v += __shfl_xor_sync(0xffffffffu, v, o);
    tot[i] = v;
  }
}

template <bool REFINE>
__global__ void __launch_bounds__(XH_WARPS * 32, 2)
xw_head_kernel(int n_maps, HeadParams hp, dinotrk_head_weights wts, int n_tiles, const float* __restrict__ norms,
               const float* __restrict__ desc_norm, const int* __restrict__ cell_frame, const int* __restrict__ cell_group,
               const int* __restrict__ cell_of, const int2* __restrict__ box_org, const int* __restrict__ stat,
               const int* __restrict__ cand, const unsigned long long* __restrict__ key1, const float* __restrict__ max2,
               const float* __restrict__ xbox, const float* __restrict__ eps_map, const int* __restrict__ grp_map0,
               const int* __restrict__ out_index, float* __restrict__ out, int* __restrict__ slow_cnt,
               int* __restrict__ slow_list, int n_groups) {
  extern __shared__ __align__(16) float xh_smem[];
  const int lane = threadIdx.x & 31, wid = __shfl_sync(0xffffffffu, (int)(threadIdx.x >> 5), 0);
  const int hf = lane >> 4, l = lane & 15;
  float* ws = xh_smem + wid * XH_PER_WARP;
  float* win = ws + hf * XH_WIN;
  float* red = ws + 2 * XH_WIN + hf * XH_RED;
  float* zb = ws + 2 * XH_WIN + 4 * XH_RED + hf * XH_ZB;
  float* racc = ws + XH_RAW + hf * XH_WIN;
  float* rfn = racc + 2 * XH_WIN;
  float w1[9], w2[9];
#pragma unroll
  for (int k = 0; k < 9; ++k) { w1[k] = wts.w1[l][k]; w2[k] = wts.w2[l][k]; }
  const float b1 = wts.b1[l];
  const int h = hp.h, w = hp.w;
  const int n_pairs = (n_maps + 1) >> 1, stride = gridDim.x * XH_WARPS;

  int pair = blockIdx.x * XH_WARPS + wid;
  XhGather gt;
  if (pair < n_pairs)
    xh_gather(gt, 2 * pair + hf, n_maps, l, h, w, hp.P, n_tiles, norms, desc_norm, cell_frame, cell_of, box_org, stat, cand,
              key1, max2, xbox, eps_map, racc, rfn);
  for (; pair < n_pairs; pair += stride) {
    const int map = 2 * pair + hf, amax = gt.amax;
    const bool exact = amax >= 0;
    const int arow = exact ? amax / w : 7, acol = exact ? amax - arow * w : 7;
    float mout = xh_window(gt, racc, rfn, win, l);
#pragma unroll
    for (int o = 8; o > 0; o >>= 1) mout = fmaxf(mout, __shfl_xor_sync(0xffffffffu, mout, o));
    const bool any = __any_sync(0xffffffffu, exact);
    const bool interior = __all_sync(0xffffffffu, !exact || (arow >= 7 && arow + 7 < h && acol >= 7 && acol + 7 < w));
    if (pair + stride < n_pairs)
      xh_gather(gt, 2 * (pair + stride) + hf, n_maps, l, h, w, hp.P, n_tiles, norms, desc_norm, cell_frame, cell_of, box_org,
                stat, cand, key1, max2, xbox, eps_map, racc, rfn);
    __syncwarp();
    if constexpr (!REFINE) {
      if (l == 0 && exact) out[(size_t)(out_index ? out_index[map] : map) * hp.out_stride] = mout;
      continue;
    }
    float zmax = 0.f;
    float tot[5] = {0.f, 0.f, 0.f, 0.f, 0.f};
    if (any) {
      if (interior) xh_refine<true>(win, red, zb, w1, b1, w2, wts.b2, arow, acol, h, w, l);
      else xh_refine<false>(win, red, zb, w1, b1, w2, wts.b2, arow, acol, h, w, l);
      __syncwarp();
      xh_sums(hp, zb, arow, acol, l, zmax, tot);
    }
    if (l == 0 && map < n_maps) {
      if (exact && head_certified(hp, wts, mout, zmax, tot)) {
        head_store_point(hp, __fdiv_rn(tot[2], tot[1]), __fdiv_rn(tot[3], tot[1]), out_index, out, map);
      } else {
        const int g = cell_group[cell_of[map]];
        const int pos = atomicAdd(slow_cnt + g, 1);
        slow_list[grp_map0[g] + pos] = map;
        atomicAdd(slow_cnt + n_groups, 1);
        if (exact) atomicAdd(slow_cnt + n_groups + 1, 1);
      }
    }
    __syncwarp();
  }
}

static int g_xw_head_window_only = 0;

int launch_xw_head(const FeatView& fv, const dinotrk_geom& g, const dinotrk_head_weights& hw, const XwCells& cells,
                   const float* desc_norm, const int* grp_map0, int n_maps, const int* out_index, float* out, int out_stride,
                   int out_mode, const XwChunk& xc, cudaStream_t st, int n_groups, const float* eps) {
  if (n_maps <= 0) return DINOTRK_OK;
  DTK_CHECK_ARG(disc_fits_box(g), "exact-window path: disc radius %d exceeds 5 tokens", g.radius);
  const HeadParams hp = make_head_params(g, hw, dinotrk_map_stride(&g), out_stride, out_mode);
  const int sms = num_sms();
  int grid = cdiv(cdiv(n_maps, 2), XH_WARPS);
  if (grid > sms * 2) grid = sms * 2;
  static PerDev<bool> attr_dev;
  bool& attr = attr_dev.get();
  if (!attr) {
    DTK_CUDA(cudaFuncSetAttribute(xw_head_kernel<true>, cudaFuncAttributeMaxDynamicSharedMemorySize, XH_SMEM));
    DTK_CUDA(cudaFuncSetAttribute(xw_head_kernel<false>, cudaFuncAttributeMaxDynamicSharedMemorySize, XH_SMEM));
    attr = true;
  }
  ProfRange pr(PROF_XW_HEAD, st);
  (g_xw_head_window_only ? xw_head_kernel<false> : xw_head_kernel<true>)<<<grid, XH_WARPS * 32, XH_SMEM, st>>>(n_maps, hp, hw, cdiv(hp.P, XW_TILE), fv.norms, desc_norm, cells.frame,
                                                       cells.group, xc.cell_of, xc.box_org, xc.stat, xc.cand, xc.key1, xc.max2,
                                                       xc.xbox, eps, grp_map0, out_index, out, xc.slow_cnt, xc.slow_list,
                                                       n_groups);
  DTK_LAUNCHED();
  return DINOTRK_OK;
}

template <bool HILO>
__global__ void __launch_bounds__(128)
xw_compact_kernel(const float4* __restrict__ desc, const uint4* __restrict__ dhi, const uint4* __restrict__ dlo,
                  const int* __restrict__ arow, const float* __restrict__ desc_norm, const int* __restrict__ out_index, int C, const int* __restrict__ grp_frame,
                  const int* __restrict__ grp_map0, int n_groups, const int* __restrict__ slow_cnt,
                  const int* __restrict__ slow_list, float4* __restrict__ c_desc, uint4* __restrict__ c_hi, uint4* __restrict__ c_lo,
                  float* __restrict__ c_norm, int* __restrict__ c_out_index, int* __restrict__ cgrp, int gcap, int row_base,
                  int grp_base) {
  __shared__ int s_g, s_pos;
  const int bb = blockIdx.x;
  if (threadIdx.x == 0) {
    int pre = 0, gsel = -1, psel = 0;
    for (int g = 0; g < n_groups; ++g) {
      const int c = slow_cnt[g];
      if (bb == 0) {
        cgrp[grp_base + g] = grp_frame[g]; cgrp[gcap + grp_base + g] = row_base + pre; cgrp[2 * gcap + grp_base + g] = c;
        cgrp[3 * gcap + grp_base + g] = row_base + pre;
      }
      if (gsel < 0 && bb < pre + c) { gsel = g; psel = bb - pre; }
      pre += c;
    }
    s_g = gsel; s_pos = psel;
  }
  __syncthreads();
  if (s_g < 0) return;
  const int b = row_base + bb;
  const int src = slow_list[grp_map0[s_g] + s_pos];
  const size_t srow = arow ? arow[src] : src;
  if (desc != nullptr)
    for (int i = threadIdx.x; i < C / 4; i += blockDim.x) c_desc[(size_t)b * (C / 4) + i] = desc[srow * (C / 4) + i];
  if (dhi != nullptr)
    for (int i = threadIdx.x; i < C / 8; i += blockDim.x) {
      if (HILO) {
        const size_t o = (size_t)b * (C / 4) + (i >> 2) * 8 + (i & 3);
        c_hi[o] = dhi[srow * (C / 8) + i];
        c_hi[o + 4] = dlo[srow * (C / 8) + i];
      } else {
        c_hi[(size_t)b * (C / 8) + i] = dhi[srow * (C / 8) + i];
        c_lo[(size_t)b * (C / 8) + i] = dlo[srow * (C / 8) + i];
      }
    }
  if (threadIdx.x == 0) { c_norm[b] = desc_norm[src]; c_out_index[b] = out_index[src]; }
}

int launch_xw_compact(const float* desc, const void* desc_hi, const void* desc_lo, const int* arow, const float* desc_norm,
                      const int* out_index, int C, const int* grp_frame, const int* grp_map0, int n_groups, int n_slow,
                      const XwChunk& xc, float* c_desc, void* c_hi, void* c_lo, float* c_norm, int* c_out_index, int* cgrp,
                      int gcap, cudaStream_t st, int row_base, int grp_base, bool hilo) {
  if (n_slow <= 0) return DINOTRK_OK;
  DTK_CHECK_ARG(!hilo || C % 32 == 0, "xw_compact: interleaved rows need C %% 32 == 0");
  ProfRange pr(PROF_MISC, st);
  (hilo ? xw_compact_kernel<true> : xw_compact_kernel<false>)<<<n_slow, 128, 0, st>>>(reinterpret_cast<const float4*>(desc), reinterpret_cast<const uint4*>(desc_hi),
                                            reinterpret_cast<const uint4*>(desc_lo), arow, desc_norm, out_index, C, grp_frame, grp_map0,
                                            n_groups, xc.slow_cnt, xc.slow_list, reinterpret_cast<float4*>(c_desc),
                                            reinterpret_cast<uint4*>(c_hi), reinterpret_cast<uint4*>(c_lo), c_norm, c_out_index, cgrp,
                                            gcap, row_base, grp_base);
  DTK_LAUNCHED();
  return DINOTRK_OK;
}

__global__ void xw_tile_prefix_kernel(const int* __restrict__ grp_m, int n_groups, int* __restrict__ tile_start) {
  const int lane = threadIdx.x;
  int base = 0;
  for (int g0 = 0; g0 < n_groups; g0 += 32) {
    const int g = g0 + lane;
    const int v = g < n_groups ? (grp_m[g] + TC2_BM - 1) / TC2_BM : 0;
    int inc = v;
#pragma unroll
    for (int o = 1; o < 32; o <<= 1) {
      const int u = __shfl_up_sync(0xffffffffu, inc, o);
      if (lane >= o) inc += u;
    }
    if (g < n_groups) tile_start[g] = base + inc - v;
    base += __shfl_sync(0xffffffffu, inc, 31);
  }
  if (lane == 0) tile_start[n_groups] = base;
}

struct XwKeysWs {
  float* rnorms; int* tile_start; unsigned* min_bits;
  XwKeysWs(Arena& ar, size_t tokens, int n_groups) {
    rnorms = ar.take<float>(tokens);
    tile_start = ar.take<int>(n_groups + 1);
    min_bits = ar.take<unsigned>(1);
  }
};

__global__ void xw_eps_kernel(const int* __restrict__ grp_frame, const int* __restrict__ grp_row0, const int* __restrict__ grp_m,
                              const float* __restrict__ rho, const float* __restrict__ rho_f, float slack, float* __restrict__ eps) {
  const int g = blockIdx.x, r0 = grp_row0[g];
  const float rf = rho_f[grp_frame[g]];
  for (int r = threadIdx.x; r < grp_m[g]; r += blockDim.x) eps[r0 + r] = xw_eps_s8(rho[r0 + r], rf, slack);
}

}

using namespace dtk;

extern "C" {

size_t dinotrk_xw_coarse_keys_workspace_bytes(int T, int n_groups, const dinotrk_geom* g) {
  return align_up(layout_end<XwKeysWs>((size_t)T * (g ? (size_t)g->h * g->w : 0), n_groups), 256) + 1024;
}

int dinotrk_xw_coarse_keys(const dinotrk_features* feat, const dinotrk_geom* g, const void* desc_hi, int desc_rows,
                           const float* desc_norm, const int* grp_frame, const int* grp_row0, const int* grp_m, int n_groups,
                           unsigned long long* key1, float* max2, void* workspace, size_t workspace_bytes, void* stream) {
  DTK_CHECK_ARG(feat && feat->norms && feat->hi && g && desc_hi && desc_norm && grp_frame && grp_row0 && grp_m && key1 && max2,
                "xw_coarse_keys: null pointer (the fp16 split of the features is required)");
  DTK_CHECK_ARG(feat->T > 0 && feat->C > 0 && feat->C % 8 == 0 && desc_rows > 0 && n_groups >= 0,
                "xw_coarse_keys: bad sizes (C must be a multiple of 8)");
  DTK_CHECK_ARG(workspace && workspace_bytes >= dinotrk_xw_coarse_keys_workspace_bytes(feat->T, n_groups, g),
                "xw_coarse_keys: workspace too small");
  if (n_groups == 0) return DINOTRK_OK;
  cudaStream_t st = (cudaStream_t)stream;
  const FeatView fv = make_view(*feat, *g);
  Arena ar(workspace);
  const XwKeysWs ws(ar, (size_t)fv.T * fv.P, n_groups);
  int rc = launch_xw_rnorms(fv, ws.rnorms, ws.min_bits, st);
  if (rc) return rc;
  {
    ProfRange pr(PROF_MISC, st);
    xw_tile_prefix_kernel<<<1, 32, 0, st>>>(grp_m, n_groups, ws.tile_start);
    DTK_LAUNCHED();
  }
  XwChunk xc{};
  xc.key1 = key1;
  xc.max2 = max2;
  return launch_xw_coarse(fv, desc_hi, desc_rows, desc_norm, grp_frame, grp_row0, grp_m, grp_row0, ws.tile_start, n_groups,
                          desc_rows / TC2_BM + n_groups, xc, st, ws.rnorms);
}

int dinotrk_xw_coarse_keys_i8(const dinotrk_features* feat, const dinotrk_geom* g, const void* desc_q8, const float* desc_fac,
                              const float* desc_rho, int desc_rows, const int* grp_frame, const int* grp_row0, const int* grp_m,
                              int n_groups, unsigned long long* key1, float* max2, float* eps, void* workspace,
                              size_t workspace_bytes, void* stream) {
  DTK_CHECK_ARG(feat && feat->norms && feat->q8 && feat->q_fac && feat->q_rho && g && desc_q8 && desc_fac && desc_rho &&
                grp_frame && grp_row0 && grp_m && key1 && max2, "xw_coarse_keys_i8: null pointer (the int8 features are required)");
  DTK_CHECK_ARG(feat->T > 0 && feat->C > 0 && feat->C % 16 == 0 && feat->C <= XW_S8_MAX_C && desc_rows > 0 && n_groups >= 0,
                "xw_coarse_keys_i8: bad sizes (C must be a multiple of 16, <= %d)", XW_S8_MAX_C);
  DTK_CHECK_ARG(workspace && workspace_bytes >= dinotrk_xw_coarse_keys_workspace_bytes(feat->T, n_groups, g),
                "xw_coarse_keys_i8: workspace too small");
  if (n_groups == 0) return DINOTRK_OK;
  cudaStream_t st = (cudaStream_t)stream;
  const FeatView fv = make_view(*feat, *g);
  Arena ar(workspace);
  const XwKeysWs ws(ar, (size_t)fv.T * fv.P, n_groups);
  {
    ProfRange pr(PROF_MISC, st);
    xw_tile_prefix_kernel<<<1, 32, 0, st>>>(grp_m, n_groups, ws.tile_start);
    DTK_LAUNCHED();
    if (eps) {
      xw_eps_kernel<<<n_groups, 128, 0, st>>>(grp_frame, grp_row0, grp_m, desc_rho, fv.q_rho, xw_s8_slack(fv.C), eps);
      DTK_LAUNCHED();
    }
  }
  XwChunk xc{};
  xc.key1 = key1;
  xc.max2 = max2;
  return launch_xw_coarse(fv, nullptr, desc_rows, nullptr, grp_frame, grp_row0, grp_m, grp_row0, ws.tile_start, n_groups,
                          desc_rows / TC2_BM + n_groups, xc, st, nullptr, desc_q8, desc_fac);
}

int dinotrk_xw_head_set_window_only(int on) {
  DTK_CHECK_ARG(on == 0 || on == 1, "xw_head_set_window_only: 0 or 1");
  g_xw_head_window_only = on;
  return DINOTRK_OK;
}

int dinotrk_xw_box_gemm_ext(const dinotrk_features* feat, const dinotrk_geom* g, const void* desc_hi, const void* desc_lo,
                            int desc_rows, const int* cell_row0, const int* cell_m, const int* cell_frame, const int* box_org,
                            const int* box_ext, int n_cells, int max_m, float* xbox, void* stream) {
  DTK_CHECK_ARG(feat && feat->hi && feat->lo && g && desc_hi && desc_lo && cell_row0 && cell_m && cell_frame && box_org && xbox,
                "xw_box_gemm: null pointer (the fp16 split of the features is required)");
  DTK_CHECK_ARG(feat->T > 0 && feat->C > 0 && feat->C % 8 == 0 && desc_rows > 0 && n_cells >= 0 && max_m > 0 &&
                max_m <= XW_MAX_CELL, "xw_box_gemm: bad sizes (C must be a multiple of 8, cells of 1..%d rows)", XW_MAX_CELL);
  DTK_CHECK_ARG(reinterpret_cast<uintptr_t>(box_org) % 8 == 0, "xw_box_gemm: box_org must be 8-byte aligned");
  DTK_CHECK_ARG(reinterpret_cast<uintptr_t>(box_ext) % 16 == 0, "xw_box_gemm: box_ext must be 16-byte aligned");
  const FeatView fv = make_view(*feat, *g);
  const XwCells cells{cell_row0, cell_row0, cell_m, cell_frame, nullptr, n_cells, max_m};
  XwChunk xc{};
  xc.box_org = reinterpret_cast<int2*>(const_cast<int*>(box_org));
  xc.box_ext = reinterpret_cast<int4*>(const_cast<int*>(box_ext));
  xc.xbox = xbox;
  return launch_xw_gemm(fv, *g, desc_hi, desc_lo, desc_rows, cells, xc, (cudaStream_t)stream);
}

int dinotrk_xw_box_gemm(const dinotrk_features* feat, const dinotrk_geom* g, const void* desc_hi, const void* desc_lo,
                        int desc_rows, const int* cell_row0, const int* cell_m, const int* cell_frame, const int* box_org,
                        int n_cells, int max_m, float* xbox, void* stream) {
  return dinotrk_xw_box_gemm_ext(feat, g, desc_hi, desc_lo, desc_rows, cell_row0, cell_m, cell_frame, box_org, nullptr, n_cells,
                                 max_m, xbox, stream);
}

}
```

### dino_tracker_b200/csrc/xwin.cuh

```cuda
#pragma once
#include <type_traits>

#include "common.cuh"
#include "corr.cuh"

namespace dtk {

constexpr float XW_EPS = 1.1e-3f;
constexpr int XW_BOX = 21;
constexpr int XW_SLACK = 3;
constexpr int XW_COLS = 448;
constexpr int XW_MAX_CELL = 128;
constexpr int XW_MAX_CAND = 4;
constexpr float XW_MIN_NORM = 1e-4f;
constexpr int XW_TILE = 128;

constexpr float XW_S8_SLACK = 3.0518e-5f;
constexpr int XW_S8_EXACT_C = 1040;
constexpr int XW_S8_MAX_C = 2048;
inline float xw_s8_slack(int C) {
  if (C <= XW_S8_EXACT_C) return XW_S8_SLACK;
  const double s = (double)XW_S8_SLACK + 3.0 * (double)((C + 15) / 16) * 0x1p-23;
  const float f = (float)s;
  return (double)f < s ? nextafterf(f, INFINITY) : f;
}
constexpr float XW_S8_RHO_MAX = 0.03f;
__device__ __forceinline__ float xw_eps_s8(float rho_d, float rho_f, float slack) {
  return __fadd_ru(__fadd_ru(rho_d, __fmul_ru(__fadd_ru(1.f, rho_d), rho_f)), slack);
}

template <class Load>
__device__ __forceinline__ float xw_quant_row(const Load& ld, int C, float norm, int8_t* __restrict__ q, float* __restrict__ fac) {
  const int lane = threadIdx.x & 31;
  float mx = 0.f;
  for (int k = 4 * lane; k < C; k += 128) {
    const float4 v = ld(k);
    mx = fmaxf(mx, fmaxf(fmaxf(fabsf(v.x), fabsf(v.y)), fmaxf(fabsf(v.z), fabsf(v.w))));
  }
#pragma unroll
  for (int o = 16; o > 0; o >>= 1) mx = fmaxf(mx, __shfl_xor_sync(0xffffffffu, mx, o));
  const float s = __fdiv_rn(mx, 127.f);
  double r2 = 0.0, x2 = 0.0;
  for (int k = 4 * lane; k < C; k += 128) {
    const float4 v = ld(k);
    const float vv[4] = {v.x, v.y, v.z, v.w};
    char4 o;
    signed char* oc = reinterpret_cast<signed char*>(&o);
#pragma unroll
    for (int e = 0; e < 4; ++e) {
      const float qf = s > 0.f ? fminf(fmaxf(rintf(__fdiv_rn(vv[e], s)), -127.f), 127.f) : 0.f;
      oc[e] = (signed char)qf;
      const double d = (double)vv[e] - (double)s * (double)qf;
      r2 = fma(d, d, r2);
      x2 = fma((double)vv[e], (double)vv[e], x2);
    }
    *reinterpret_cast<char4*>(q + k) = o;
  }
#pragma unroll
  for (int o = 16; o > 0; o >>= 1) {
    r2 += __shfl_xor_sync(0xffffffffu, r2, o);
    x2 += __shfl_xor_sync(0xffffffffu, x2, o);
  }
  if (lane == 0) *fac = __fdiv_rn(s, fmaxf(norm, XW_MIN_NORM));
  return x2 > 0.0 ? __double2float_ru(__ddiv_ru(__dsqrt_ru(r2), __dsqrt_rd(x2))) : 0.f;
}

__host__ __device__ inline int xw_col(int by, int bx) { return by * XW_BOX + bx; }

struct XwChunk {
  unsigned long long* key1;
  float* max2;
  int* cand;
  int* pinfo;
  int* stat;
  int* cell_of;
  int2* box_org;
  int4* box_ext;
  float* xbox;
  int* slow_cnt;
  int* slow_list;
  XwChunk() = default;
  XwChunk(Arena& ar, size_t maps, size_t cells, int n_tiles, int n_groups) {
    key1 = ar.take<unsigned long long>(maps * n_tiles);
    max2 = ar.take<float>(maps * n_tiles);
    cand = ar.take<int>(maps * XW_MAX_CAND);
    stat = ar.take<int>(maps);
    pinfo = ar.take<int>(maps);
    cell_of = ar.take<int>(maps);
    slow_list = ar.take<int>(maps);
    box_org = ar.take<int2>(cells);
    box_ext = ar.take<int4>(cells);
    xbox = ar.take<float>(maps * XW_COLS);
    slow_cnt = ar.take<int>((size_t)n_groups + 4);
  }
};

struct XwCells {
  const int* row0;
  const int* arow;
  const int* m;
  const int* frame;
  const int* group;
  int n_cells, max_m;
};

int launch_xw_coarse(const FeatView& fv, const void* desc_hi, int desc_rows, const float* desc_norm, const int* grp_frame,
                     const int* grp_row0, const int* grp_m, const int* grp_map0, const int* tile_start, int n_groups,
                     int max_tiles, const XwChunk& xc, cudaStream_t st, const float* rnorms, const void* desc_q8 = nullptr,
                     const float* desc_fac = nullptr);
int launch_xw_rnorms(const FeatView& fv, float* rnorms, unsigned* min_bits, cudaStream_t st);
int launch_xw_plan(const XwCells& cells, const float* desc_norm, int n_groups, const dinotrk_geom& g, const XwChunk& xc,
                   cudaStream_t st, int n_maps, float min_norm, const float* eps);
int launch_xw_gemm(const FeatView& fv, const dinotrk_geom& g, const void* desc_hi, const void* desc_lo, int desc_rows,
                   const XwCells& cells, const XwChunk& xc, cudaStream_t st);
int launch_xw_head(const FeatView& fv, const dinotrk_geom& g, const dinotrk_head_weights& hw, const XwCells& cells,
                   const float* desc_norm, const int* grp_map0, int n_maps, const int* out_index, float* out, int out_stride,
                   int out_mode, const XwChunk& xc, cudaStream_t st, int n_groups, const float* eps);
int launch_xw_compact(const float* desc, const void* desc_hi, const void* desc_lo, const int* arow, const float* desc_norm,
                      const int* out_index, int C, const int* grp_frame, const int* grp_map0, int n_groups, int n_slow,
                      const XwChunk& xc, float* c_desc, void* c_hi, void* c_lo, float* c_norm, int* c_out_index, int* cgrp,
                      int gcap, cudaStream_t st, int row_base = 0, int grp_base = 0, bool hilo = false);

}
```

Measured before the change: 12560.

## Move cosine normalization into window GEMM epilogue and precompute head records

The window GEMM epilogue now turns raw dot products into clamped cosine values, using descriptor and feature norms loaded per tile. The plan kernels precompute per-candidate outside-max terms and a compact per-map rectangle record, replacing the stat flags. The head kernel then prefetches these 16-byte records with cp.async and double buffers them instead of gathering norms, keys and maxima itself. The cand kernel grid is also sized from queried occupancy. This shifts work from the head into the GEMM and plan stages and adds memory for mterm and rect.

```diff
diff --git a/dino_tracker_b200/csrc/inference.cu b/dino_tracker_b200/csrc/inference.cu
--- a/dino_tracker_b200/csrc/inference.cu
+++ b/dino_tracker_b200/csrc/inference.cu
@@ -765,9 +765,8 @@
                                cm.n_groups, cm.used / TC2_BM_ROWS + cm.n_groups, x.xc, st, ws.d_rnorms,
                                choice.s8 ? ws.u_q8 : nullptr, ws.u_fac))) return rc;
     if ((rc = launch_xw_plan(cells, x.norm, cm.n_groups, c.g, x.xc, st, cm.used, split_min_norm(c.C), eps))) return rc;
-    if ((rc = launch_xw_gemm(c.fv, c.g, ws.u_hi, ws.u_lo, (int)ws.xw_rows, cells, x.xc, st))) return rc;
-    if ((rc = launch_xw_head(c.fv, c.g, c.hw, cells, x.norm, gp.map0, cm.used, x.out_index, anchors, 2, 0, x.xc, st, cm.n_groups,
-                             eps)))
+    if ((rc = launch_xw_gemm(c.fv, c.g, ws.u_hi, ws.u_lo, (int)ws.xw_rows, cells, x.xc, st, x.norm))) return rc;
+    if ((rc = launch_xw_head(c.g, c.hw, cells, gp.map0, cm.used, x.out_index, anchors, 2, 0, x.xc, st, cm.n_groups)))
       return rc;
     DTK_CUDA(cudaMemcpyAsync(xa->host_cnt + XW_CNT_CHUNK * (k % XW_RING), x.xc.slow_cnt + cm.n_groups, XW_CNT_CHUNK * sizeof(int),
                              cudaMemcpyDeviceToHost, st));
diff --git a/dino_tracker_b200/csrc/xwin.cu b/dino_tracker_b200/csrc/xwin.cu
--- a/dino_tracker_b200/csrc/xwin.cu
+++ b/dino_tracker_b200/csrc/xwin.cu
@@ -158,9 +158,10 @@
 constexpr int PLAN_WARPS = 8;
 template <int KPL>
 __global__ void __launch_bounds__(PLAN_WARPS * 32)
-xw_cand_kernel(int n_maps, const float* __restrict__ desc_norm, float min_norm, int n_groups, int n_tiles,
+xw_cand_kernel(int n_maps, const float* __restrict__ desc_norm, float min_norm, int n_groups, int n_tiles, int w,
                const unsigned long long* __restrict__ key1, const float* __restrict__ eps_map,
-               const float* __restrict__ max2, int* __restrict__ cand, int* __restrict__ pinfo, int* __restrict__ slow_cnt) {
+               const float* __restrict__ max2, int* __restrict__ cand, float* __restrict__ mterm, int* __restrict__ pinfo,
+               int* __restrict__ slow_cnt) {
   const int lane = threadIdx.x & 31;
   const int gw = blockIdx.x * PLAN_WARPS + (threadIdx.x >> 5), nw = gridDim.x * PLAN_WARPS;
   if (gw == 0)
@@ -198,14 +199,34 @@
       ncand += __popc(cm);
     }
     amb = amb || ncand > XW_MAX_CAND || !(gmax > 4.f * eps) || !(desc_norm[map] >= min_norm);
+    if (lane == 0) pinfo[map] = amb ? -1 - ptok : ptok;
+    if (!amb) {
+      __syncwarp();
+#pragma unroll 1
+      for (int s = 0; s < ncand; ++s) {
+        const int cs = ncand == 1 ? ptok : cand[(size_t)map * XW_MAX_CAND + s];
+        const int cr = cs / w, cc = cs - cr * w;
+        float mt = 0.f;
+#pragma unroll
+        for (int q = 0; q < KPL; ++q)
+          if (lane + 32 * q < n_tiles) {
+            const int tk = 0x7fffffff - (int)(kk[q] & 0xffffffffu), tr = tk / w, tcn = tk - tr * w;
+            const bool in_core = abs(tr - cr) <= 3 && abs(tcn - cc) <= 3;
+            mt = fmaxf(mt, (in_core ? v2[q] : __uint_as_float((unsigned)(kk[q] >> 32))) + eps);
+          }
+#pragma unroll
+        for (int o = 16; o > 0; o >>= 1) mt = fmaxf(mt, __shfl_xor_sync(0xffffffffu, mt, o));
+        if (lane == 0) mterm[(size_t)map * XW_MAX_CAND + s] = mt;
+      }
+    }
     if (lane >= ncand && lane < XW_MAX_CAND) cand[(size_t)map * XW_MAX_CAND + lane] = -1;
-    if (lane == 0) pinfo[map] = amb ? -1 - ptok : ptok;
   }
 }
 
 __global__ void __launch_bounds__(PLAN_WARPS * 32)
-xw_cell_kernel(XwCells cells, int w, const int* __restrict__ cand, const int* __restrict__ pinfo, int* __restrict__ stat,
-               int* __restrict__ cell_of, int2* __restrict__ box_org, int4* __restrict__ box_ext, int* __restrict__ box_cnt) {
+xw_cell_kernel(XwCells cells, int h, int w, const int* __restrict__ cand, const int* __restrict__ pinfo,
+               XwRect* __restrict__ rect, int* __restrict__ cell_of, int2* __restrict__ box_org, int4* __restrict__ box_ext,
+               int* __restrict__ box_cnt) {
   __shared__ short s_r[PLAN_WARPS][XW_MAX_CELL], s_c[PLAN_WARPS][XW_MAX_CELL];
   __shared__ unsigned char s_ok[PLAN_WARPS][XW_MAX_CELL];
   const int lane = threadIdx.x & 31, wid = threadIdx.x >> 5;
@@ -246,6 +267,7 @@
         med_c = max(med_c, __shfl_xor_sync(0xffffffffu, med_c, o));
       }
     }
+    const int org_r = med_r - XW_BOX / 2, org_c = med_c - XW_BOX / 2, fo = cells.frame[cell] * (h * w);
     int n_fit = 0, lo_r = INT_MAX, hi_r = INT_MIN, lo_c = INT_MAX, hi_c = INT_MIN;
     for (int r = lane; r < m; r += 32) {
       const int map = row0 + r;
@@ -262,7 +284,13 @@
             mr0 = min(mr0, tr); mr1 = max(mr1, tr); mc0 = min(mc0, tc_); mc1 = max(mc1, tc_);
           }
       }
-      stat[map] = fit ? 0 : 1;
+      XwRect rc{-1, 0, 0, 0, 0, 0};
+      if (fit) {
+        const int r0 = max(mr0 - WM / 2, 0), c0 = max(mc0 - WM / 2, 0);
+        rc = XwRect{fo, (short)r0, (short)c0, (short)(min(mr1 + WM / 2, h - 1) - r0 + 1),
+                    (short)(min(mc1 + WM / 2, w - 1) - c0 + 1), xw_col(r0 - org_r, c0 - org_c)};
+      }
+      rect[map] = rc;
       n_fit += fit ? 1 : 0;
       if (fit) { lo_r = min(lo_r, mr0); hi_r = max(hi_r, mr1); lo_c = min(lo_c, mc0); hi_c = max(hi_c, mc1); }
     }
@@ -273,7 +301,6 @@
       lo_c = min(lo_c, __shfl_xor_sync(0xffffffffu, lo_c, o)); hi_c = max(hi_c, __shfl_xor_sync(0xffffffffu, hi_c, o));
     }
     if (lane == 0) {
-      const int org_r = med_r - XW_BOX / 2, org_c = med_c - XW_BOX / 2;
       box_org[cell] = n_fit > 0 ? make_int2(org_r, org_c) : make_int2(0, INT_MIN);
       if (n_fit > 0) {
         const int4 e = make_int4(lo_r - WM / 2 - org_r, lo_c - WM / 2 - org_c, hi_r - lo_r + WM, hi_c - lo_c + WM);
@@ -294,16 +321,19 @@
   static_assert(DTK_GRID_MAX_TOKENS <= 256 * XW_TILE, "xw_cand_kernel keeps at most 8 keys per lane");
   DTK_CHECK_ARG(cells.max_m <= XW_MAX_CELL, "exact-window path: cell of %d rows", cells.max_m);
   if (cells.n_cells <= 0 || n_maps <= 0) return DINOTRK_OK;
+  auto cand_kernel = n_tiles <= 64 ? xw_cand_kernel<2> : n_tiles <= 128 ? xw_cand_kernel<4> : xw_cand_kernel<8>;
+  int resident = 0;
+  DTK_CUDA(cudaOccupancyMaxActiveBlocksPerMultiprocessor(&resident, cand_kernel, PLAN_WARPS * 32, 0));
   ProfRange pr(PROF_XW_PLAN, st);
   int grid = cdiv(n_maps, PLAN_WARPS);
-  if (grid > num_sms() * 8) grid = num_sms() * 8;
-  auto cand_kernel = n_tiles <= 64 ? xw_cand_kernel<2> : n_tiles <= 128 ? xw_cand_kernel<4> : xw_cand_kernel<8>;
-  cand_kernel<<<grid, PLAN_WARPS * 32, 0, st>>>(n_maps, desc_norm, min_norm, n_groups, n_tiles, xc.key1, eps, xc.max2, xc.cand, xc.pinfo, xc.slow_cnt);
+  if (grid > num_sms() * resident) grid = num_sms() * resident;
+  cand_kernel<<<grid, PLAN_WARPS * 32, 0, st>>>(n_maps, desc_norm, min_norm, n_groups, n_tiles, g.w, xc.key1, eps, xc.max2,
+                                                xc.cand, xc.mterm, xc.pinfo, xc.slow_cnt);
   DTK_LAUNCHED();
   grid = cdiv(cells.n_cells, PLAN_WARPS);
   if (grid > num_sms() * 8) grid = num_sms() * 8;
-  xw_cell_kernel<<<grid, PLAN_WARPS * 32, 0, st>>>(cells, g.w, xc.cand, xc.pinfo, xc.stat, xc.cell_of, xc.box_org, xc.box_ext,
-                                                   xc.slow_cnt + n_groups + 2);
+  xw_cell_kernel<<<grid, PLAN_WARPS * 32, 0, st>>>(cells, g.h, g.w, xc.cand, xc.pinfo, xc.rect, xc.cell_of, xc.box_org,
+                                                   xc.box_ext, xc.slow_cnt + n_groups + 2);
   DTK_LAUNCHED();
   return DINOTRK_OK;
 }
@@ -357,13 +387,26 @@
   __device__ __forceinline__ int row(int i) const { return y + i * (bh / n) + min(i, bh % n); }
 };
 
+struct XwVal { const float* dnorm; const float* fnorm; int h, w; };
+
 template <int MB, bool HILO>
 __device__ __forceinline__ void xw_part(uint8_t* smem, uint64_t* full, uint64_t* empty, float* epi, int& stage, int& phase, int KB,
                                         uint32_t d_off, uint32_t t_off, uint32_t t_half, float* __restrict__ xbox, int map0,
-                                        int r0, int m, int ntok, int bw, int col0) {
+                                        int r0, int m, int ntok, int bw, int col0, const XwVal& val, int gr0, int gc0) {
   using Cfg = XwCfg<MB, HILO>;
   constexpr int N = XW_PART_TOK;
   const int warp = threadIdx.x >> 5, lane = threadIdx.x & 31, t = threadIdx.x & 127;
+  const int rw = r0 + (warp & 3) * 16;
+  const int nr = min(m - rw, XW_EPI_ROWS);
+  float dnl = 0.f, fn[N / 32];
+  if (val.dnorm) {
+    dnl = lane < nr ? __ldg(val.dnorm + map0 + rw + lane) : 0.f;
+#pragma unroll
+    for (int q = 0; q < N / 32; ++q) {
+      const int j = 32 * q + lane, y = j / bw, gr = gr0 + y, gc = gc0 + j - y * bw;
+      fn[q] = j < ntok && gr >= 0 && gr < val.h && gc >= 0 && gc < val.w ? __ldg(val.fnorm + gr * val.w + gc) : -1.f;
+    }
+  }
   float acc[N / 2];
 #pragma unroll
   for (int i = 0; i < N / 2; ++i) acc[i] = 0.f;
@@ -392,10 +435,9 @@
   tc::wgmma_wait<0>();
   tc::reg_fence(acc);
   if (prev >= 0 && t == 0) tc::mbar_arrive(&empty[prev]);
-  const int rw = r0 + (warp & 3) * 16, fr = lane >> 2, fc = 2 * (lane & 3);
+  const int fr = lane >> 2, fc = 2 * (lane & 3);
   float* buf = epi + (warp & 7) * XW_EPI_ROWS * XW_EPI_PITCH;
   float* dst = xbox + (size_t)(map0 + rw) * XW_COLS + col0;
-  const int nr = min(m - rw, XW_EPI_ROWS);
 #pragma unroll
   for (int q = 0; q < N / 32; ++q) {
     if (32 * q >= ntok || nr <= 0) break;
@@ -407,8 +449,13 @@
             make_float2(acc[4 * (4 * q + ii) + 2 * h], acc[4 * (4 * q + ii) + 2 * h + 1]);
     __syncwarp();
     const int j = 32 * q + lane, y = j / bw, off = y * XW_BOX + (j - y * bw);
-    if (j < ntok)
-      for (int k = 0; k < nr; ++k) dst[(size_t)k * XW_COLS + off] = buf[k * XW_EPI_PITCH + lane];
+    const bool in = fn[q] >= 0.f;
+    for (int k = 0; k < nr; ++k) {
+      float v = buf[k * XW_EPI_PITCH + lane];
+      const float dn = __shfl_sync(0xffffffffu, dnl, k);
+      if (val.dnorm) v = in ? fmaxf(corr_cos(v, dn, fn[q]), 0.f) : 0.f;
+      if (j < ntok) dst[(size_t)k * XW_COLS + off] = v;
+    }
     __syncwarp();
   }
 }
@@ -417,7 +464,8 @@
 __global__ void __launch_bounds__(TC_THREADS, 1)
 xw_gemm_kernel(const __grid_constant__ CUtensorMap tmD_hi, const __grid_constant__ CUtensorMap tmD_lo,
                const __grid_constant__ XwTokMaps<HILO> tok, XwCells cells, const int2* __restrict__ box_org,
-               const int4* __restrict__ box_ext, float* __restrict__ xbox, int K) {
+               const int4* __restrict__ box_ext, float* __restrict__ xbox, int K, const float* __restrict__ desc_norm,
+               const float* __restrict__ norms, int h, int w) {
   using Cfg = XwCfg<MB, HILO>;
   extern __shared__ uint8_t smem_raw[];
   uint8_t* smem = reinterpret_cast<uint8_t*>((reinterpret_cast<uintptr_t>(smem_raw) + 1023) & ~(uintptr_t)1023);
@@ -470,9 +518,9 @@
     tc::regs_alloc<232>();
     const int cw = wg - 1;
     int stage = 0, phase = 0;
-    struct Meta { bool skip; XwExt<MB> e; int m, map0; };
+    struct Meta { int2 org; XwExt<MB> e; int m, map0, frame; };
     auto meta = [&](int cell) {
-      return Meta{box_org[cell].y == INT_MIN, XwExt<MB>(box_ext, cell), cells.m[cell], cells.row0[cell]};
+      return Meta{box_org[cell], XwExt<MB>(box_ext, cell), cells.m[cell], cells.row0[cell], cells.frame[cell]};
     };
     Meta cur;
     if (blockIdx.x < cells.n_cells) cur = meta(blockIdx.x);
@@ -481,15 +529,18 @@
       if (cell + gridDim.x < cells.n_cells) nxt = meta(cell + gridDim.x);
       const XwExt<MB>& e = cur.e;
       const int m = cur.m, map0 = cur.map0;
-      if (!cur.skip)
+      const XwVal val{desc_norm, desc_norm ? norms + (size_t)cur.frame * h * w : nullptr, h, w};
+      if (cur.org.y != INT_MIN)
         for (int p0 = 0; p0 < e.n; p0 += Cfg::kParts) {
           if constexpr (MB == 64) {
             const int p = p0 + cw;
             xw_part<MB, HILO>(smem, full, empty, epi, stage, phase, KB, 0, Cfg::kTokOff + cw * Cfg::kBoxes * Cfg::kSlotBytes,
-                              Cfg::kSlotBytes, xbox, map0, 0, m, e.rows(p) * e.bw, e.bw, xw_col(e.row(p), e.x));
+                              Cfg::kSlotBytes, xbox, map0, 0, m, e.rows(p) * e.bw, e.bw, xw_col(e.row(p), e.x), val,
+                              cur.org.x + e.row(p), cur.org.y + e.x);
           } else {
             xw_part<MB, HILO>(smem, full, empty, epi, stage, phase, KB, cw * 64 * Cfg::kRow, Cfg::kTokOff, Cfg::kSlotBytes,
-                              xbox, map0, 64 * cw, m, e.rows(p0) * e.bw, e.bw, xw_col(e.row(p0), e.x));
+                              xbox, map0, 64 * cw, m, e.rows(p0) * e.bw, e.bw, xw_col(e.row(p0), e.x), val,
+                              cur.org.x + e.row(p0), cur.org.y + e.x);
           }
         }
       cur = nxt;
@@ -526,7 +577,7 @@
 
 template <int MB, bool HILO>
 static int run_xw_gemm(const FeatView& fv, const dinotrk_geom& g, const CUtensorMap (&tmD)[2], const XwCells& cells,
-                       const XwChunk& xc, cudaStream_t st) {
+                       const XwChunk& xc, cudaStream_t st, const float* desc_norm) {
   const XwTokMaps<HILO>* tok;
   if (int rc = xw_tok_maps<HILO>(fv, g, tok)) return rc;
   static PerDev<bool> attr_dev;
@@ -539,13 +590,14 @@
   const int grid = cells.n_cells < sms ? cells.n_cells : sms;
   ProfRange pr(PROF_XW_GEMM, st);
   xw_gemm_kernel<MB, HILO><<<grid, TC_THREADS, XwCfg<MB, HILO>::kSmem, st>>>(tmD[0], tmD[1], *tok, cells, xc.box_org, xc.box_ext,
-                                                                              xc.xbox, fv.C);
+                                                                              xc.xbox, fv.C, desc_norm, fv.norms, g.h,
+                                                                              g.w);
   DTK_LAUNCHED();
   return DINOTRK_OK;
 }
 
 int launch_xw_gemm(const FeatView& fv, const dinotrk_geom& g, const void* desc_hi, const void* desc_lo, int desc_rows,
-                   const XwCells& cells, const XwChunk& xc, cudaStream_t st) {
+                   const XwCells& cells, const XwChunk& xc, cudaStream_t st, const float* desc_norm) {
   if (cells.n_cells <= 0) return DINOTRK_OK;
   DTK_CHECK_ARG(fv.C % 8 == 0 && cells.max_m <= XW_MAX_CELL, "exact-window GEMM: bad sizes");
   const bool small = cells.max_m <= 64, hilo = fv.hilo != nullptr;
@@ -554,8 +606,11 @@
   int rc;
   if ((rc = make_tmap_2d(&tmD[0], desc_hi, desc_rows, fv.C, small ? 64 : 128, BK, TMAP_F16, 0, SW))) return rc;
   if ((rc = make_tmap_2d(&tmD[1], desc_lo, desc_rows, fv.C, small ? 64 : 128, BK, TMAP_F16, 0, SW))) return rc;
-  if (hilo) return small ? run_xw_gemm<64, true>(fv, g, tmD, cells, xc, st) : run_xw_gemm<128, true>(fv, g, tmD, cells, xc, st);
-  return small ? run_xw_gemm<64, false>(fv, g, tmD, cells, xc, st) : run_xw_gemm<128, false>(fv, g, tmD, cells, xc, st);
+  if (hilo)
+    return small ? run_xw_gemm<64, true>(fv, g, tmD, cells, xc, st, desc_norm)
+                 : run_xw_gemm<128, true>(fv, g, tmD, cells, xc, st, desc_norm);
+  return small ? run_xw_gemm<64, false>(fv, g, tmD, cells, xc, st, desc_norm)
+               : run_xw_gemm<128, false>(fv, g, tmD, cells, xc, st, desc_norm);
 }
 
 constexpr int XH_WARPS = 8;
@@ -564,101 +619,73 @@
 constexpr int XH_RP = 20;
 constexpr int XH_RED = 240;
 constexpr int XH_ZB = 128;
+constexpr int XH_RECT = XW_BOX * XW_BOX;
+constexpr int XH_REC = 12;
 constexpr int XH_RAW = 2 * XH_WIN + 4 * XH_RED + 2 * XH_ZB;
-constexpr int XH_PER_WARP = XH_RAW + 4 * XH_WIN;
+constexpr int XH_RECS = XH_RAW + (2 * XH_RECT + 3) / 4 * 4;
+constexpr int XH_PER_WARP = XH_RECS + 4 * XH_REC;
 constexpr int XH_SMEM = XH_WARPS * XH_PER_WARP * 4;
 static_assert(XH_WIN % 32 == 16 && XH_RED % 32 == 16 && WB * XH_RP <= XH_RED && WB * WB <= XH_ZB, "head buffer layout");
-
-constexpr int XH_KEYS = 4;
-
-struct XhGather {
-  int amax;
-  float dn, mout;
-  unsigned ok;
-};
+static_assert(XH_RECS % 4 == 0 && XH_REC % 4 == 0 && XH_PER_WARP % 4 == 0 && sizeof(XwRect) == 16,
+              "record slots must be 16-byte aligned");
+static_assert(2 * (XH_SMEM + 1024) <= 228 * 1024, "two head blocks per SM");
 
 __device__ __forceinline__ void xh_cp4(float* dst, const float* src) {
   asm volatile("cp.async.ca.shared.global [%0], [%1], 4;\n" ::"r"((unsigned)__cvta_generic_to_shared(dst)), "l"(src) : "memory");
 }
+__device__ __forceinline__ void xh_cp16(void* dst, const void* src) {
+  asm volatile("cp.async.cg.shared.global [%0], [%1], 16;\n" ::"r"((unsigned)__cvta_generic_to_shared(dst)), "l"(src) : "memory");
+}
 __device__ __forceinline__ void xh_cp_wait() { asm volatile("cp.async.wait_all;\n" ::: "memory"); }
 
-__device__ __forceinline__ void xh_gather(XhGather& gt, int map, int n_maps, int l, int h, int w, int P, int n_tiles,
-                                          const float* __restrict__ norms, const float* __restrict__ desc_norm,
-                                          const int* __restrict__ cell_frame, const int* __restrict__ cell_of,
-                                          const int2* __restrict__ box_org, const int* __restrict__ stat,
-                                          const int* __restrict__ cand, const unsigned long long* __restrict__ key1,
-                                          const float* __restrict__ max2, const float* __restrict__ xbox,
-                                          const float* __restrict__ eps_map, float* __restrict__ racc, float* __restrict__ rfn) {
-  gt.amax = -1;
-  gt.ok = 0;
-  if (map >= n_maps) return;
-  const int st = __ldg(stat + map), cell = __ldg(cell_of + map);
-  const float dn = __ldg(desc_norm + map);
-  const int4 cd = __ldg(reinterpret_cast<const int4*>(cand) + map);
-  const float eps = eps_map ? __ldg(eps_map + map) : XW_EPS;
-  const unsigned long long* k1 = key1 + (size_t)map * n_tiles;
-  const float* k2 = max2 + (size_t)map * n_tiles;
-  unsigned long long kk[XH_KEYS];
-  float kv2[XH_KEYS];
-#pragma unroll
-  for (int q = 0; q < XH_KEYS; ++q) {
-    const int t = l + 16 * q;
-    kk[q] = t < n_tiles ? __ldg(k1 + t) : 0ull;
-    kv2[q] = t < n_tiles ? __ldg(k2 + t) : 0.f;
-  }
-  if (st != 0) return;
-  const int2 org = __ldg(box_org + cell);
-  const float* fn = norms + (size_t)__ldg(cell_frame + cell) * P;
-  const float* xr = xbox + (size_t)map * XW_COLS;
+__device__ __forceinline__ void xh_fetch(float* slot, int map, int n_maps, int l, const XwRect* __restrict__ rect,
+                                         const int* __restrict__ cand, const float* __restrict__ mterm) {
+  if (map >= n_maps) {
+    if (l == 0) reinterpret_cast<XwRect*>(slot)->fo = -1;
+  } else if (l == 0) {
+    xh_cp16(slot, rect + map);
+  } else if (l == 1) {
+    xh_cp16(slot + 4, cand + (size_t)map * XW_MAX_CAND);
+  } else if (l == 2) {
+    xh_cp16(slot + 8, mterm + (size_t)map * XW_MAX_CAND);
+  }
+}
+
+__device__ __forceinline__ void xh_issue(const float* slot, int map, int l, const float* __restrict__ xbox,
+                                         float* __restrict__ rv) {
+  const XwRect rc = *reinterpret_cast<const XwRect*>(slot);
+  if (rc.fo < 0) return;
+  const float* xr = xbox + (size_t)map * XW_COLS + rc.col0;
+  for (int c = l; c < rc.rw; c += 16)
+    for (int y = 0; y < rc.rh; ++y) xh_cp4(rv + y * XW_BOX + c, xr + y * XW_BOX + c);
+}
+
+__device__ __forceinline__ float xh_window(const float* slot, const float* __restrict__ rv, float* __restrict__ win, int l,
+                                           int h, int w, int& amax) {
+  const XwRect rc = *reinterpret_cast<const XwRect*>(slot);
+  const int4 cd = *reinterpret_cast<const int4*>(slot + 4);
+  const float4 mt = *reinterpret_cast<const float4*>(slot + 8);
   const int ct[4] = {cd.x, cd.y, cd.z, cd.w};
-  float best = -1.f;
-  int amax = -1;
-#pragma unroll
-  for (int q = 0; q < XW_MAX_CAND; ++q)
-    if (ct[q] >= 0) {
-      const int tr = ct[q] / w, tcn = ct[q] - tr * w;
-      const float v = fmaxf(corr_cos(__ldg(xr + xw_col(tr - org.x, tcn - org.y)), dn, __ldg(fn + ct[q])), 0.f);
-      if (v > best || (v == best && ct[q] < amax)) { best = v; amax = ct[q]; }
-    }
-  const int arow = amax / w, acol = amax - arow * w;
-  float mout = 0.f;
-  auto fold = [&](unsigned long long k, float m2) {
-    const int tk = 0x7fffffff - (int)(k & 0xffffffffu);
-    const int tr = tk / w, tcn = tk - tr * w;
-    const bool in_core = abs(tr - arow) <= 3 && abs(tcn - acol) <= 3;
-    mout = fmaxf(mout, (in_core ? m2 : __uint_as_float((unsigned)(k >> 32))) + eps);
-  };
-#pragma unroll
-  for (int q = 0; q < XH_KEYS; ++q)
-    if (l + 16 * q < n_tiles) fold(kk[q], kv2[q]);
-  for (int t = l + 16 * XH_KEYS; t < n_tiles; t += 16) fold(__ldg(k1 + t), __ldg(k2 + t));
-  const int c = acol - 7 + l;
-  const bool col_in = l < WM && c >= 0 && c < w;
-  unsigned ok = 0;
+  const float mtv[4] = {mt.x, mt.y, mt.z, mt.w};
+  amax = -1;
+  float best = -1.f, mout = 0.f;
+  if (rc.fo >= 0) {
+#pragma unroll
+    for (int q = 0; q < XW_MAX_CAND; ++q)
+      if (ct[q] >= 0) {
+        const int tr = ct[q] / w, tcn = ct[q] - tr * w;
+        const float v = rv[(tr - rc.r0) * XW_BOX + (tcn - rc.c0)];
+        if (v > best || (v == best && ct[q] < amax)) { best = v; amax = ct[q]; mout = mtv[q]; }
+      }
+  }
+  const int arow = amax / w, acol = amax - arow * w, c = acol - 7 + l;
+  const bool col_in = amax >= 0 && l < WM && c >= 0 && c < w;
 #pragma unroll
   for (int y = 0; y < WM; ++y) {
     const int r = arow - 7 + y;
+    float v = 0.f;
     if (col_in && r >= 0 && r < h) {
-      xh_cp4(racc + y * XH_WP + l, xr + xw_col(r - org.x, c - org.y));
-      xh_cp4(rfn + y * XH_WP + l, fn + r * w + c);
-      ok |= 1u << y;
-    }
-  }
-  gt.amax = amax;
-  gt.dn = dn;
-  gt.mout = mout;
-  gt.ok = ok;
-}
-
-__device__ __forceinline__ float xh_window(const XhGather& gt, const float* __restrict__ racc, const float* __restrict__ rfn,
-                                           float* __restrict__ win, int l) {
-  xh_cp_wait();
-  float mout = gt.mout;
-#pragma unroll
-  for (int y = 0; y < WM; ++y) {
-    float v = 0.f;
-    if ((gt.ok >> y) & 1u) {
-      v = fmaxf(corr_cos(racc[y * XH_WP + l], gt.dn, rfn[y * XH_WP + l]), 0.f);
+      v = rv[(r - rc.r0) * XW_BOX + (c - rc.c0)];
       if (!(abs(y - 7) <= 3 && abs(l - 7) <= 3)) mout = fmaxf(mout, v);
     }
     win[y * XH_WP + l] = v;
@@ -779,13 +806,11 @@
 
 template <bool REFINE>
 __global__ void __launch_bounds__(XH_WARPS * 32, 2)
-xw_head_kernel(int n_maps, HeadParams hp, dinotrk_head_weights wts, int n_tiles, const float* __restrict__ norms,
-               const float* __restrict__ desc_norm, const int* __restrict__ cell_frame, const int* __restrict__ cell_group,
-               const int* __restrict__ cell_of, const int2* __restrict__ box_org, const int* __restrict__ stat,
-               const int* __restrict__ cand, const unsigned long long* __restrict__ key1, const float* __restrict__ max2,
-               const float* __restrict__ xbox, const float* __restrict__ eps_map, const int* __restrict__ grp_map0,
-               const int* __restrict__ out_index, float* __restrict__ out, int* __restrict__ slow_cnt,
-               int* __restrict__ slow_list, int n_groups) {
+xw_head_kernel(int n_maps, HeadParams hp, dinotrk_head_weights wts, const int* __restrict__ cell_group,
+               const int* __restrict__ cell_of,
+               const XwRect* __restrict__ rect, const int* __restrict__ cand, const float* __restrict__ mterm,
+               const float* __restrict__ xbox, const int* __restrict__ grp_map0, const int* __restrict__ out_index,
+               float* __restrict__ out, int* __restrict__ slow_cnt, int* __restrict__ slow_list, int n_groups) {
   extern __shared__ __align__(16) float xh_smem[];
   const int lane = threadIdx.x & 31, wid = __shfl_sync(0xffffffffu, (int)(threadIdx.x >> 5), 0);
   const int hf = lane >> 4, l = lane & 15;
@@ -793,8 +818,8 @@
   float* win = ws + hf * XH_WIN;
   float* red = ws + 2 * XH_WIN + hf * XH_RED;
   float* zb = ws + 2 * XH_WIN + 4 * XH_RED + hf * XH_ZB;
-  float* racc = ws + XH_RAW + hf * XH_WIN;
-  float* rfn = racc + 2 * XH_WIN;
+  float* rv = ws + XH_RAW + hf * XH_RECT;
+  float* const slot0 = ws + XH_RECS + hf * XH_REC;
   float w1[9], w2[9];
 #pragma unroll
   for (int k = 0; k < 9; ++k) { w1[k] = wts.w1[l][k]; w2[k] = wts.w2[l][k]; }
@@ -803,23 +828,26 @@
   const int n_pairs = (n_maps + 1) >> 1, stride = gridDim.x * XH_WARPS;
 
   int pair = blockIdx.x * XH_WARPS + wid;
-  XhGather gt;
-  if (pair < n_pairs)
-    xh_gather(gt, 2 * pair + hf, n_maps, l, h, w, hp.P, n_tiles, norms, desc_norm, cell_frame, cell_of, box_org, stat, cand,
-              key1, max2, xbox, eps_map, racc, rfn);
-  for (; pair < n_pairs; pair += stride) {
-    const int map = 2 * pair + hf, amax = gt.amax;
+  if (pair < n_pairs) xh_fetch(slot0, 2 * pair + hf, n_maps, l, rect, cand, mterm);
+  if (pair + stride < n_pairs) xh_fetch(slot0 + 2 * XH_REC, 2 * (pair + stride) + hf, n_maps, l, rect, cand, mterm);
+  xh_cp_wait();
+  __syncwarp();
+  if (pair < n_pairs) xh_issue(slot0, 2 * pair + hf, l, xbox, rv);
+  for (int k = 0; pair < n_pairs; pair += stride, k ^= 1) {
+    const int map = 2 * pair + hf;
+    xh_cp_wait();
+    __syncwarp();
+    int amax;
+    float mout = xh_window(slot0 + 2 * XH_REC * k, rv, win, l, h, w, amax);
     const bool exact = amax >= 0;
     const int arow = exact ? amax / w : 7, acol = exact ? amax - arow * w : 7;
-    float mout = xh_window(gt, racc, rfn, win, l);
 #pragma unroll
     for (int o = 8; o > 0; o >>= 1) mout = fmaxf(mout, __shfl_xor_sync(0xffffffffu, mout, o));
     const bool any = __any_sync(0xffffffffu, exact);
     const bool interior = __all_sync(0xffffffffu, !exact || (arow >= 7 && arow + 7 < h && acol >= 7 && acol + 7 < w));
-    if (pair + stride < n_pairs)
-      xh_gather(gt, 2 * (pair + stride) + hf, n_maps, l, h, w, hp.P, n_tiles, norms, desc_norm, cell_frame, cell_of, box_org,
-                stat, cand, key1, max2, xbox, eps_map, racc, rfn);
     __syncwarp();
+    if (pair + stride < n_pairs) xh_issue(slot0 + 2 * XH_REC * (k ^ 1), 2 * (pair + stride) + hf, l, xbox, rv);
+    if (pair + 2 * stride < n_pairs) xh_fetch(slot0 + 2 * XH_REC * k, 2 * (pair + 2 * stride) + hf, n_maps, l, rect, cand, mterm);
     if constexpr (!REFINE) {
       if (l == 0 && exact) out[(size_t)(out_index ? out_index[map] : map) * hp.out_stride] = mout;
       continue;
@@ -849,9 +877,9 @@
 
 static int g_xw_head_window_only = 0;
 
-int launch_xw_head(const FeatView& fv, const dinotrk_geom& g, const dinotrk_head_weights& hw, const XwCells& cells,
-                   const float* desc_norm, const int* grp_map0, int n_maps, const int* out_index, float* out, int out_stride,
-                   int out_mode, const XwChunk& xc, cudaStream_t st, int n_groups, const float* eps) {
+int launch_xw_head(const dinotrk_geom& g, const dinotrk_head_weights& hw, const XwCells& cells, const int* grp_map0,
+                   int n_maps, const int* out_index, float* out, int out_stride, int out_mode, const XwChunk& xc,
+                   cudaStream_t st, int n_groups) {
   if (n_maps <= 0) return DINOTRK_OK;
   DTK_CHECK_ARG(disc_fits_box(g), "exact-window path: disc radius %d exceeds 5 tokens", g.radius);
   const HeadParams hp = make_head_params(g, hw, dinotrk_map_stride(&g), out_stride, out_mode);
@@ -866,10 +894,9 @@
     attr = true;
   }
   ProfRange pr(PROF_XW_HEAD, st);
-  (g_xw_head_window_only ? xw_head_kernel<false> : xw_head_kernel<true>)<<<grid, XH_WARPS * 32, XH_SMEM, st>>>(n_maps, hp, hw, cdiv(hp.P, XW_TILE), fv.norms, desc_norm, cells.frame,
-                                                       cells.group, xc.cell_of, xc.box_org, xc.stat, xc.cand, xc.key1, xc.max2,
-                                                       xc.xbox, eps, grp_map0, out_index, out, xc.slow_cnt, xc.slow_list,
-                                                       n_groups);
+  (g_xw_head_window_only ? xw_head_kernel<false> : xw_head_kernel<true>)<<<grid, XH_WARPS * 32, XH_SMEM, st>>>(
+      n_maps, hp, hw, cells.group, xc.cell_of, xc.rect, xc.cand, xc.mterm, xc.xbox, grp_map0, out_index,
+      out, xc.slow_cnt, xc.slow_list, n_groups);
   DTK_LAUNCHED();
   return DINOTRK_OK;
 }
@@ -1058,7 +1085,7 @@
   xc.box_org = reinterpret_cast<int2*>(const_cast<int*>(box_org));
   xc.box_ext = reinterpret_cast<int4*>(const_cast<int*>(box_ext));
   xc.xbox = xbox;
-  return launch_xw_gemm(fv, *g, desc_hi, desc_lo, desc_rows, cells, xc, (cudaStream_t)stream);
+  return launch_xw_gemm(fv, *g, desc_hi, desc_lo, desc_rows, cells, xc, (cudaStream_t)stream, nullptr);
 }
 
 int dinotrk_xw_box_gemm(const dinotrk_features* feat, const dinotrk_geom* g, const void* desc_hi, const void* desc_lo,
diff --git a/dino_tracker_b200/csrc/xwin.cuh b/dino_tracker_b200/csrc/xwin.cuh
--- a/dino_tracker_b200/csrc/xwin.cuh
+++ b/dino_tracker_b200/csrc/xwin.cuh
@@ -67,12 +67,19 @@
 
 __host__ __device__ inline int xw_col(int by, int bx) { return by * XW_BOX + bx; }
 
+struct alignas(16) XwRect {
+  int fo;
+  short r0, c0, rh, rw;
+  int col0;
+};
+
 struct XwChunk {
   unsigned long long* key1;
   float* max2;
   int* cand;
+  float* mterm;
   int* pinfo;
-  int* stat;
+  XwRect* rect;
   int* cell_of;
   int2* box_org;
   int4* box_ext;
@@ -84,7 +91,8 @@
     key1 = ar.take<unsigned long long>(maps * n_tiles);
     max2 = ar.take<float>(maps * n_tiles);
     cand = ar.take<int>(maps * XW_MAX_CAND);
-    stat = ar.take<int>(maps);
+    mterm = ar.take<float>(maps * XW_MAX_CAND);
+    rect = ar.take<XwRect>(maps);
     pinfo = ar.take<int>(maps);
     cell_of = ar.take<int>(maps);
     slow_list = ar.take<int>(maps);
@@ -112,10 +120,9 @@
 int launch_xw_plan(const XwCells& cells, const float* desc_norm, int n_groups, const dinotrk_geom& g, const XwChunk& xc,
                    cudaStream_t st, int n_maps, float min_norm, const float* eps);
 int launch_xw_gemm(const FeatView& fv, const dinotrk_geom& g, const void* desc_hi, const void* desc_lo, int desc_rows,
-                   const XwCells& cells, const XwChunk& xc, cudaStream_t st);
-int launch_xw_head(const FeatView& fv, const dinotrk_geom& g, const dinotrk_head_weights& hw, const XwCells& cells,
-                   const float* desc_norm, const int* grp_map0, int n_maps, const int* out_index, float* out, int out_stride,
-                   int out_mode, const XwChunk& xc, cudaStream_t st, int n_groups, const float* eps);
+                   const XwCells& cells, const XwChunk& xc, cudaStream_t st, const float* desc_norm);
+int launch_xw_head(const dinotrk_geom& g, const dinotrk_head_weights& hw, const XwCells& cells, const int* grp_map0,
+                   int n_maps, const int* out_index, float* out, int out_stride, int out_mode, const XwChunk& xc, cudaStream_t st, int n_groups);
 int launch_xw_compact(const float* desc, const void* desc_hi, const void* desc_lo, const int* arow, const float* desc_norm,
                       const int* out_index, int C, const int* grp_frame, const int* grp_map0, int n_groups, int n_slow,
                       const XwChunk& xc, float* c_desc, void* c_hi, void* c_lo, float* c_norm, int* c_out_index, int* cgrp,
```

Measured after the change: 12610 (median of 6 runs). About the same (+0.4%).
